# joesharratt1229/DT4Image_Restoration

Hardware: AMD Instinct MI355X
Metric: pnp_admm_iterations_per_sec (higher is better)
Workload: dtype f32

## Files before the change

dt4image_restoration_amd/_lib.py:

```python
from __future__ import annotations

import ctypes as C
import os

_HERE = os.path.dirname(os.path.abspath(__file__))
LIB_PATH = os.environ.get("PNP_LIB_PATH") or os.path.join(_HERE, "csrc", "libpnpadmm.so")

PNP_FLAG_PROFILE = 1
PNP_FLAG_NO_DENOISER = 2
PNP_FLAG_KEEP_STAGES = 4
PNP_FLAG_BF16_CONVS = 8
PNP_FLAG_PROFILE_LAYERS = 16
PNP_SSIM_CLAMP_X = 1
PNP_RES_COLS = 6
PNP_RES_DELTA = 1
PNP_RES_DC = 2
RESIDUAL_COLUMNS = ("primal", "dx", "dz", "du", "delta", "dc")
PNP_MC_MAX_COILS = 32
PNP_MC_MAX_CG = 64
PNP_CC_MAX_COILS = 64
PNP_PW_MAX_COILS = 64
PNP_ESPIRIT_MAX_COILS = 16
PNP_ESPIRIT_MAX_KSIZE = 8
PNP_ESPIRIT_MAX_N = 512
PNP_TV_MAX_ITERS = 64
PNP_PRIOR_UNET = 0
PNP_PRIOR_TV = 1
PRIORS = {"unet": PNP_PRIOR_UNET, "tv": PNP_PRIOR_TV}
PNP_SENS_BOX = 0
PNP_SENS_HANN = 1
SENS_WINDOWS = {"box": PNP_SENS_BOX, "hann": PNP_SENS_HANN}
PROFILE_CLASSES = 6
PROFILE_CLASS_NAMES = ("conv3x3_mfma", "conv_first", "conv_last", "fft_rows", "fft_cols_prox", "other")
N_LAYERS = 28


class pnp_config(C.Structure):
    _fields_ = [("n", C.c_int32), ("h", C.c_int32), ("w", C.c_int32), ("device", C.c_int32), ("flags", C.c_int32)]


_vp, _fp, _u8p = C.c_void_p, C.c_void_p, C.c_void_p

SIGNATURES = {
    "pnp_create": (C.c_int, [C.POINTER(pnp_config), C.POINTER(C.c_void_p)]),
    "pnp_destroy": (C.c_int, [C.c_void_p]),
    "pnp_last_error": (C.c_char_p, []),
    "pnp_version": (C.c_char_p, []),
    "pnp_load_unet_weights": (C.c_int, [C.c_void_p, C.c_void_p, C.c_size_t]),
    "pnp_reset": (C.c_int, [C.c_void_p, _fp, _fp, _u8p, C.c_int, _fp, _fp, _fp, _vp]),
    "pnp_set_kspace": (C.c_int, [C.c_void_p, _fp, _u8p, C.c_int, _vp]),
    "pnp_step": (C.c_int, [C.c_void_p, _fp, _fp, _fp, _fp, _fp, _fp, _fp, _u8p, _vp]),
    "pnp_denoise": (C.c_int, [C.c_void_p, _fp, _fp, _fp, _vp]),
    "pnp_tv_denoise": (C.c_int, [C.c_void_p, _fp, _fp, C.c_int, _fp, _vp]),
    "pnp_set_prior": (C.c_int, [C.c_void_p, C.c_int, C.c_double, C.c_int]),
    "pnp_get_prior": (C.c_int, [C.c_void_p, C.POINTER(C.c_int), C.POINTER(C.c_double), C.POINTER(C.c_int)]),
    "pnp_fft2c": (C.c_int, [C.c_void_p, _fp, _fp, C.c_int, C.c_int, C.c_int, C.c_int, _vp]),
    "pnp_prox_dual": (C.c_int, [C.c_void_p, _fp, _fp, _fp, _fp, _fp, _vp]),
    "pnp_psnr": (C.c_int, [C.c_void_p, _fp, _fp, _fp, _vp]),
    "pnp_ssim": (C.c_int, [C.c_void_p, _fp, _fp, C.c_float, C.c_float, C.c_float, C.c_int, C.c_int, _fp, _fp, _vp]),
    "pnp_residuals": (C.c_int, [C.c_void_p, _fp, _fp, _fp, _vp, C.c_int, _fp, _vp]),
    "pnp_acquire": (C.c_int, [C.c_void_p, _fp, _u8p, C.c_int, C.c_double, C.c_uint64, C.c_int, _fp, _fp, _fp, _vp]),
    "pnp_set_kspace_mc": (C.c_int, [C.c_void_p, _fp, _fp, C.c_int, C.c_int, _u8p, C.c_int, C.c_int, _vp]),
    "pnp_reset_mc": (C.c_int, [C.c_void_p, _fp, _fp, _fp, C.c_int, C.c_int, _u8p, C.c_int, C.c_int, _fp, _fp, _fp, _vp]),
    "pnp_mc_coils": (C.c_int, [C.c_void_p]),
    "pnp_mc_cg_residual": (C.c_int, [C.c_void_p, _fp, _vp]),
    "pnp_mc_normal": (C.c_int, [C.c_void_p, _fp, _fp, _fp, _vp]),
    "pnp_acquire_mc": (C.c_int, [C.c_void_p, _fp, _fp, C.c_int, C.c_int, _u8p, C.c_int, C.c_double, C.c_uint64, C.c_int, _fp, _fp, _fp, _vp]),
    "pnp_estimate_sens": (C.c_int, [C.c_void_p, _fp, C.c_int, C.c_int, C.c_int, C.c_int, C.c_double, C.c_int, _fp, _fp, _vp]),
    "pnp_coil_compress_matrix": (C.c_int, [C.c_void_p, _fp, C.c_int, C.c_int, C.c_int, C.c_int, _fp, _fp, _fp, _vp]),
    "pnp_coil_compress_apply": (C.c_int, [C.c_void_p, _fp, C.c_int, _fp, C.c_int, C.c_int, _fp, _vp]),
    "pnp_noise_cov": (C.c_int, [C.c_void_p, _fp, C.c_int, C.c_int, C.c_int, C.c_int, _fp, _vp]),
    "pnp_whiten_matrix": (C.c_int, [C.c_void_p, _fp, C.c_int, C.c_int, C.c_int, _fp, _fp, _fp, _vp]),
    "pnp_whiten_apply": (C.c_int, [C.c_void_p, _fp, C.c_int, _fp, C.c_int, _fp, _vp]),
    "pnp_espirit_sens": (C.c_int, [C.c_void_p, _fp, C.c_int, C.c_int, C.c_int, C.c_int, C.c_double, C.c_double, C.c_int, C.c_int, C.c_double,
                                  C.c_int, _fp, _fp, _fp, _vp, _vp]),
    "pnp_snapshot_bytes": (C.c_size_t, [C.c_void_p]),
    "pnp_snapshot": (C.c_int, [C.c_void_p, _fp, _fp, _fp, _fp, _vp, _vp]),
    "pnp_restore": (C.c_int, [C.c_void_p, _vp, _fp, _fp, _fp, _fp, _vp]),
    "pnp_unet_read_stage": (C.c_int, [C.c_void_p, C.c_int, _fp, C.POINTER(C.c_int), C.POINTER(C.c_int),
                                      C.POINTER(C.c_int), _vp]),
    "pnp_profile_reset": (C.c_int, [C.c_void_p]),
    "pnp_profile_collect": (C.c_int, [C.c_void_p, C.POINTER(C.c_double), C.POINTER(C.c_int64)]),
    "pnp_profile_layers": (C.c_int, [C.c_void_p, C.POINTER(C.c_double), C.POINTER(C.c_int64)]),
    "pnp_conv_algorithms": (C.c_int, [C.c_void_p, C.POINTER(C.c_int32)]),
    "pnp_bf16_weight_terms": (C.c_int, [C.c_void_p]),
    "pnp_workspace_bytes": (C.c_size_t, [C.c_void_p]),
}

_lib = None


class PnPError(RuntimeError):
    pass


def load() -> C.CDLL:
    global _lib
    if _lib is not None:
        return _lib
    if not os.path.exists(LIB_PATH):
        raise PnPError(f"{LIB_PATH} not found: build it with `python -c 'import __graft_entry__ as g; g.build()'` "
                       f"or `make -C {os.path.dirname(LIB_PATH)}`; there is no CPU fallback")
    lib = C.CDLL(LIB_PATH)
    for name, (res, args) in SIGNATURES.items():
        fn = getattr(lib, name)
        fn.restype = res
        fn.argtypes = args
    _lib = lib
    return lib


def check(rc: int, what: str) -> None:
    if rc != 0:
        msg = load().pnp_last_error()
        raise PnPError(f"{what} failed ({rc}): {msg.decode() if msg else '?'}")
```

dt4image_restoration_amd/csrc/conv_kernels.hip:

```cpp
#include "pnp_internal.h"
#include "conv_staging.h"
#include <cstring>
#include <cstdlib>

namespace pnp {



const LayerSpec kLayers[N_LAYERS] = {
    {2, 32, 3, 0, SRC_SIGMA, 0},    {32, 32, 3, 0, SRC_PLAIN, 0},   {32, 32, 3, 0, SRC_PLAIN, 0},
    {32, 64, 3, 1, SRC_POOL, 0},    {64, 64, 3, 1, SRC_PLAIN, 0},   {64, 64, 3, 1, SRC_PLAIN, 0},
    {64, 128, 3, 2, SRC_POOL, 0},   {128, 128, 3, 2, SRC_PLAIN, 0}, {128, 128, 3, 2, SRC_PLAIN, 0},
    {128, 256, 3, 3, SRC_POOL, 0},  {256, 256, 3, 3, SRC_PLAIN, 0}, {256, 256, 3, 3, SRC_PLAIN, 0},
    {256, 512, 3, 4, SRC_POOL, 0},  {512, 512, 3, 4, SRC_PLAIN, 0}, {512, 512, 3, 4, SRC_PLAIN, 0},
    {768, 256, 3, 3, SRC_UPCAT, 256}, {256, 256, 3, 3, SRC_PLAIN, 0}, {256, 256, 3, 3, SRC_PLAIN, 0},
    {384, 128, 3, 2, SRC_UPCAT, 128}, {128, 128, 3, 2, SRC_PLAIN, 0}, {128, 128, 3, 2, SRC_PLAIN, 0},
    {192, 64, 3, 1, SRC_UPCAT, 64},  {64, 64, 3, 1, SRC_PLAIN, 0},   {64, 64, 3, 1, SRC_PLAIN, 0},
    {96, 32, 3, 0, SRC_UPCAT, 32},   {32, 32, 3, 0, SRC_PLAIN, 0},   {32, 32, 3, 0, SRC_PLAIN, 0},
    {32, 1, 1, 0, SRC_PLAIN, 0},
};

ConvPlan conv3x3_plan(int N, int H, int W, int Cin, int Cout, bool bf16, int src_mode, bool allow_ws) {
    ConvPlan p{};
    p.tw = W >= 32 ? 32 : (W >= 16 ? 16 : 8);
// ... 553 lines not shown
                for (unsigned z0 = 0; z0 < nz; z0 += 4) {
                    float4 q[4][4];
#pragma unroll
                    for (int k = 0; k < 4; ++k) {
                        const unsigned z = z0 + k < nz ? z0 + k : nz - 1;
#pragma unroll
                        for (int j = 0; j < 4; ++j)
                            q[k][j] = __builtin_bit_cast(float4, __builtin_amdgcn_raw_buffer_load_b128(prsrc, e[j] * 4u, (int)(z * pstride), 16));
                    }
#pragma unroll
                    for (int k = 0; k < 4; ++k)
                        if (z0 + k < nz) {
#pragma unroll
                            for (int j = 0; j < 4; ++j) { sum[j].x += q[k][j].x; sum[j].y += q[k][j].y; sum[j].z += q[k][j].z; sum[j].w += q[k][j].w; }
                        }
                }
#pragma unroll
                for (int j = 0; j < 4; ++j) {
                    if (!ok[j]) continue;
                    float4 v = sum[j];
                    v.x = fmaxf(v.x, kLeaky * v.x); v.y = fmaxf(v.y, kLeaky * v.y);
                    v.z = fmaxf(v.z, kLeaky * v.z); v.w = fmaxf(v.w, kLeaky * v.w);
                    *reinterpret_cast<float4*>(a.dst + e[j]) = v;
                }
            }
        }
    }
}

__global__ __launch_bounds__(256) void splitk_reduce_kernel(const float* __restrict__ partial, const float* __restrict__ bias,
                                                            float* __restrict__ dst, const float* __restrict__ tact,
                                                            size_t plane4, int splitk, int cout4, size_t slice4) {
    for (size_t i = (size_t)blockIdx.x * 256 + threadIdx.x; i < plane4; i += (size_t)gridDim.x * 256) {
        if (tact != nullptr && tact[i / slice4] > 0.5f) continue;
        float4 s = reinterpret_cast<const float4*>(bias)[i % cout4];
        for (int z0 = 0; z0 < splitk; z0 += 8) {
            float4 p[8];
#pragma unroll
            for (int k = 0; k < 8; ++k) p[k] = reinterpret_cast<const float4*>(partial)[(size_t)(z0 + k < splitk ? z0 + k : splitk - 1) * plane4 + i];
#pragma unroll
            for (int k = 0; k < 8; ++k)
                if (z0 + k < splitk) { s.x += p[k].x; s.y += p[k].y; s.z += p[k].z; s.w += p[k].w; }
        }
        s.x = fmaxf(s.x, kLeaky * s.x); s.y = fmaxf(s.y, kLeaky * s.y);
        s.z = fmaxf(s.z, kLeaky * s.z); s.w = fmaxf(s.w, kLeaky * s.w);
        reinterpret_cast<float4*>(dst)[i] = s;
    }
}

template <int TW, int MT, int NT, int WM, int WN, int CK, int SRC, bool SPLITK, int BF16>
static hipError_t launch_inst(const ConvArgs& a, const ConvPlan& p, hipStream_t s) {
    constexpr int WPS = (MT * NT <= 2 && SRC != SRC_UPCAT) ? 3 : (MT * NT <= 8 ? 2 : 1);
    constexpr int WPS16 = (MT * NT <= 2 && BF16 == 2) ? 3 : WPS;
    dim3 grid((unsigned)(p.tiles_x * p.tiles_y * a.N), (unsigned)(a.Cout / p.bn), (unsigned)p.splitk);
    constexpr bool CAN16 = BF16 != 0 && !SPLITK && MT == 2 && NT == 1 && WM == 4 && CK == 32 && SRC != SRC_POOL;
    if constexpr (CAN16) {
        if (a.act16 & 1) {
            hipLaunchKernelGGL((conv3x3_mfma_kernel<TW, MT, NT, WM, WN, CK, SRC, WPS16, SPLITK, BF16, true>), grid, dim3(256), 0, s, a);
            return hipGetLastError();
        }
    }
    if (a.act16 != 0) return hipErrorInvalidValue;
    hipLaunchKernelGGL((conv3x3_mfma_kernel<TW, MT, NT, WM, WN, CK, SRC, WPS, SPLITK, BF16, false>), grid, dim3(256), 0, s, a);
    return hipGetLastError();
}

template <int TW, int MT, int NT, int WM, int WN, int CK, bool SPLITK, int BF16>
static hipError_t launch_cfg(const ConvArgs& a, const ConvPlan& p, int src_mode, hipStream_t s) {
    switch (src_mode) {
        case SRC_PLAIN: return launch_inst<TW, MT, NT, WM, WN, CK, SRC_PLAIN, SPLITK, BF16>(a, p, s);
        case SRC_POOL:  return launch_inst<TW, MT, NT, WM, WN, CK, SRC_POOL, SPLITK, BF16>(a, p, s);
        case SRC_UPCAT: return launch_inst<TW, MT, NT, WM, WN, CK, SRC_UPCAT, SPLITK, BF16>(a, p, s);
        default: return hipErrorInvalidValue;
    }
}

template <int TW, int BF16>
static hipError_t launch_tw(const ConvArgs& a, const ConvPlan& p, int src_mode, hipStream_t s) {
    if constexpr (BF16 == 0) {
        if (p.mt == 1 && p.wn == 4) return launch_cfg<TW, 1, 1, 1, 4, 16, true, 0>(a, p, src_mode, s);
        if (p.mt == 1 && p.wn == 2) return launch_cfg<TW, 1, 1, 2, 2, 16, true, 0>(a, p, src_mode, s);
    }
    if (p.mt == 2 && p.wn == 4) return launch_cfg<TW, 2, 1, 1, 4, 32, true, BF16>(a, p, src_mode, s);
    if (p.mt == 2 && p.wn == 2) return launch_cfg<TW, 2, 1, 2, 2, 32, true, BF16>(a, p, src_mode, s);
    if constexpr (BF16 == 0) {
        if (p.nt == 1 && p.mt == 1) return launch_cfg<TW, 1, 1, 4, 1, 32, false, 0>(a, p, src_mode, s);
    }
    if (p.nt == 1) return launch_cfg<TW, 2, 1, 4, 1, 32, false, BF16>(a, p, src_mode, s);
    if (p.nt == 2 && p.wn == 1) return launch_cfg<TW, 4, 2, 4, 1, 16, false, BF16>(a, p, src_mode, s);
    if (p.nt == 2) return launch_cfg<TW, 4, 2, 2, 2, 32, false, BF16>(a, p, src_mode, s);
    if constexpr (BF16 != 0) return hipErrorInvalidValue;
    else return launch_cfg<TW, 4, 4, 2, 2, 32, false, 0>(a, p, src_mode, s);
}

hipError_t launch_conv3x3(const ConvArgs& a0, const ConvPlan& p, int src_mode, hipStream_t s) {
    if (a0.Cin % 32 != 0 || a0.Cout % 32 != 0 || (a0.Cout > 64 && a0.Cout % 128 != 0)) return hipErrorInvalidValue;
    if (!conv3x3_tensor_fits(a0.N, a0.H, a0.W, a0.Cin, a0.Cout)) return hipErrorInvalidValue;
    if (p.ws) return launch_conv3x3_bf16ws(a0, p, src_mode, s);
    ConvArgs a = a0;
    a.tilesX = p.tiles_x;
    a.tilesY = p.tiles_y;
    const bool split = p.mt <= 2 && p.wn >= 2;
    if (split && a.partial == nullptr) return hipErrorInvalidValue;
    if (!split || (size_t)p.tiles_x * p.tiles_y * a.N * (a.Cout / p.bn) > 4096) a.arrive = nullptr;
    hipError_t e;
    if (a.bf16 == 2) {
        if (p.tw == 32) e = launch_tw<32, 2>(a, p, src_mode, s);
        else if (p.tw == 16) e = launch_tw<16, 2>(a, p, src_mode, s);
        else e = launch_tw<8, 2>(a, p, src_mode, s);
    } else if (a.bf16 == 1) {
        if (p.tw == 32) e = launch_tw<32, 1>(a, p, src_mode, s);
        else if (p.tw == 16) e = launch_tw<16, 1>(a, p, src_mode, s);
        else e = launch_tw<8, 1>(a, p, src_mode, s);
    } else {
        if (p.tw == 32) e = launch_tw<32, 0>(a, p, src_mode, s);
        else if (p.tw == 16) e = launch_tw<16, 0>(a, p, src_mode, s);
        else e = launch_tw<8, 0>(a, p, src_mode, s);
    }
    if (e != hipSuccess || !split || a.arrive != nullptr) return e;
    const size_t plane4 = (size_t)a.N * a.H * a.W * a.Cout / 4;
    unsigned blocks = (unsigned)((plane4 + 255) / 256);
    if (blocks > 2048u) blocks = 2048u;
    hipLaunchKernelGGL(splitk_reduce_kernel, dim3(blocks), dim3(256), 0, s, a.partial, a.bias, a.dst, a.tact, plane4,
                       p.splitk, a.Cout / 4, (size_t)a.H * a.W * a.Cout / 4);
    return hipGetLastError();
}

bool conv3x3_tensor_fits(int N, int H, int W, int Cin, int Cout) {
    (void)Cin;
    return (size_t)N * H * W * (size_t)Cout * 4 < ((size_t)1 << 31);
}

bool conv3x3_pooled_output_ok(const ConvPlan& p) {
    return p.splitk == 1 && p.mt <= 2 && p.nt == 1 && p.wm == 4;
}

size_t conv3x3_partial_floats(const ConvPlan& p, int N, int H, int W, int Cout) {
    return (p.mt <= 2 && p.wn >= 2) ? (size_t)p.splitk * N * H * W * Cout : 0;
}

Tuning tuning_from_env() {
    Tuning t;
    if (const char* v = getenv("PNP_WINO_MIN_CIN")) t.wino_min_cin = atoi(v);
    if (const char* v = getenv("PNP_WINO_MIN_BLOCKS")) t.wino_min_blocks = atol(v);
    t.wino_big = getenv("PNP_WINO_BIG_GROUPS") != nullptr;
    t.wino_small = getenv("PNP_WINO_SMALL_GROUPS") != nullptr;
    t.no_wino = getenv("PNP_NO_WINOGRAD") != nullptr;
    if (const char* v = getenv("PNP_WINO_F4_MIN_CIN")) t.f4_min_cin = atoi(v);
    t.no_f4 = getenv("PNP_NO_WINO_F4") != nullptr;
    t.no_f4_phased = getenv("PNP_NO_WINO_F4_PHASED") != nullptr;
    t.no_f4_fused_last = getenv("PNP_NO_F4_FUSED_LAST") != nullptr;
    t.no_f4_fused_first = getenv("PNP_NO_F4_FUSED_FIRST") != nullptr;
    if (const char* v = getenv("PNP_WINO_F4_MT16")) t.f4_mt16 = atoi(v);
    if (const char* v = getenv("PNP_WINO_F4_ORDER")) t.f4_order = atoi(v) != 0;
    t.bf16_f32_acts = getenv("PNP_BF16_F32_ACTS") != nullptr;
    t.bf16_no_ws = getenv("PNP_BF16_NO_WS") != nullptr;
    t.bf16_w1 = getenv("PNP_BF16_W1") != nullptr;
    t.bf16_no_holdhi = getenv("PNP_BF16_NO_HOLDHI") != nullptr;
    t.fft_xcd = getenv("PNP_FFT_XCD") != nullptr && atoi(getenv("PNP_FFT_XCD")) != 0;
    if (const char* v = getenv("PNP_SPLITK_INLAUNCH")) t.splitk_inlaunch = atoi(v);
    if (const char* v = getenv("PNP_SLICE128_MIN_N")) t.slice128_min_n = atoi(v);
    return t;
}

hipError_t raise_lds_cap(const void* fn, int bytes, DeviceOnce& once) {
    int dev = 0;
    hipError_t e = hipGetDevice(&dev);
    if (e != hipSuccess) return e;
    const uint64_t bit = 1ull << (dev & 63);
    if (once.mask.load(std::memory_order_relaxed) & bit) return hipSuccess;
    e = hipFuncSetAttribute(fn, hipFuncAttributeMaxDynamicSharedMemorySize, bytes);
    if (e != hipSuccess) return e;
    once.mask.fetch_or(bit, std::memory_order_relaxed);
    return hipSuccess;
}

__global__ __launch_bounds__(256) void conv_first_kernel(const float* __restrict__ ximg, const float2* __restrict__ z,
                                                         const float2* __restrict__ u, const float* __restrict__ sigma,
                                                         const float* __restrict__ tact, const float* __restrict__ w,
                                                         const float* __restrict__ bias, float* __restrict__ dst,
                                                         int N, int H, int W, int tilesX, int tilesY, int TYG, int dst16) {
    constexpr int TH = 8, TW = 32, PW = TW + 2, PH = TH + 2;
    __shared__ float dt[2][PH][PW + 1];
    __shared__ float mt[2][PH][PW + 1];
    const int groupsY = (tilesY + TYG - 1) / TYG;
    int bt = blockIdx.x;
    const int tx0 = (bt % tilesX) * TW;
    bt /= tilesX;
    const int tyg = bt % groupsY;
    const int n = bt / groupsY;
    if (tact != nullptr && tact[n] > 0.5f) return;
    auto stage = [&](int buf, int ty0) {
        for (int i = threadIdx.x; i < PH * PW; i += 256) {
            const int py = i / PW, px = i % PW;
            const int gy = ty0 + py - 1, gx = tx0 + px - 1;
            float d = 0.f, m = 0.f;
            if (gy >= 0 && gy < H && gx >= 0 && gx < W) {
                const size_t q = ((size_t)n * H + gy) * W + gx;
                d = ximg != nullptr ? ximg[q] : (z[q].x - u[q].x);
                m = 1.f;
            }
            dt[buf][py][px] = d;
            mt[buf][py][px] = m;
        }
    };
    const int t_first = tyg * TYG, t_last = min(t_first + TYG, tilesY);
    stage(0, t_first * TH);
    const int cg = threadIdx.x & 7, col = threadIdx.x >> 3;
    float wd[4][9], ws[4][9], br[4], brs[4];
    const float sg = sigma[n];
#pragma unroll
    for (int j = 0; j < 4; ++j) {
        br[j] = bias[cg * 4 + j];
        brs[j] = br[j];
#pragma unroll
        for (int k = 0; k < 9; ++k) {
            wd[j][k] = w[(cg * 4 + j) * 18 + k];
            ws[j][k] = w[(cg * 4 + j) * 18 + 9 + k] * sg;
            brs[j] += ws[j][k];
        }
    }
    const int gx = tx0 + col;
    for (int t = t_first; t < t_last; ++t) {
        const int buf = (t - t_first) & 1, ty0 = t * TH;
        const bool interior = tx0 > 0 && tx0 + TW < W && ty0 > 0 && ty0 + TH < H;
        __syncthreads();
        if (t + 1 < t_last) stage(buf ^ 1, ty0 + TH);
        float d[3][3], m[3][3];
#pragma unroll
        for (int r = 0; r < 2; ++r)
#pragma unroll
            for (int c = 0; c < 3; ++c) { d[r + 1][c] = dt[buf][r][col + c]; m[r + 1][c] = mt[buf][r][col + c]; }
#pragma unroll
        for (int row = 0; row < TH; ++row) {
#pragma unroll
            for (int c = 0; c < 3; ++c) {
                d[0][c] = d[1][c]; d[1][c] = d[2][c]; d[2][c] = dt[buf][row + 2][col + c];
                m[0][c] = m[1][c]; m[1][c] = m[2][c]; m[2][c] = mt[buf][row + 2][col + c];
            }
            float acc[4];
            if (interior) {
#pragma unroll
                for (int j = 0; j < 4; ++j) acc[j] = brs[j];
#pragma unroll
                for (int ky = 0; ky < 3; ++ky)
#pragma unroll
                    for (int kx = 0; kx < 3; ++kx)
#pragma unroll
                        for (int j = 0; j < 4; ++j) acc[j] = fmaf(wd[j][ky * 3 + kx], d[ky][kx], acc[j]);
            } else {
#pragma unroll
                for (int j = 0; j < 4; ++j) acc[j] = br[j];
#pragma unroll
                for (int ky = 0; ky < 3; ++ky)
#pragma unroll
                    for (int kx = 0; kx < 3; ++kx)
#pragma unroll
                        for (int j = 0; j < 4; ++j) {
                            acc[j] = fmaf(wd[j][ky * 3 + kx], d[ky][kx], acc[j]);
                            acc[j] = fmaf(ws[j][ky * 3 + kx], m[ky][kx], acc[j]);
                        }
            }
            const int gy = ty0 + row;
            if (gy < H && gx < W) {
                float4 o;
                o.x = fmaxf(acc[0], kLeaky * acc[0]);
                o.y = fmaxf(acc[1], kLeaky * acc[1]);
                o.z = fmaxf(acc[2], kLeaky * acc[2]);
                o.w = fmaxf(acc[3], kLeaky * acc[3]);
                if (dst16) {
                    uint2 o16;
                    o16.x = __builtin_bit_cast(unsigned, __builtin_convertvector((f32x2){o.x, o.y}, bf16x2));
                    o16.y = __builtin_bit_cast(unsigned, __builtin_convertvector((f32x2){o.z, o.w}, bf16x2));
                    *reinterpret_cast<uint2*>(reinterpret_cast<uint16_t*>(dst) + (((size_t)n * H + gy) * W + gx) * 32 + cg * 4) = o16;
                } else {
                    *reinterpret_cast<float4*>(dst + (((size_t)n * H + gy) * W + gx) * 32 + cg * 4) = o;
                }
            }
        }
    }
}

hipError_t launch_conv_first(const float* ximg, const float2* z, const float2* u, const float* sigma,
                             const float* tact, const float* w, const float* bias, float* dst, int N, int H, int W,
                             hipStream_t s, bool dst_bf16) {
    const int tilesX = (W + 31) / 32, tilesY = (H + 7) / 8;
    int tyg = 8;
    while (tyg > 1 && (long)tilesX * ((tilesY + tyg - 1) / tyg) * N < 512) tyg >>= 1;
    const int groupsY = (tilesY + tyg - 1) / tyg;
    hipLaunchKernelGGL(conv_first_kernel, dim3((unsigned)(tilesX * groupsY * N)), dim3(256), 0, s, ximg, z, u, sigma, tact, w,
                       bias, dst, N, H, W, tilesX, tilesY, tyg, dst_bf16 ? 1 : 0);
    return hipGetLastError();
}

__global__ __launch_bounds__(256) void conv_last_kernel(const float* __restrict__ act, const float* __restrict__ ximg,
                                                        const float2* __restrict__ z, const float2* __restrict__ u,
                                                        const float* __restrict__ tact, const float* __restrict__ w,
                                                        const float* __restrict__ bias, float* __restrict__ out,
                                                        int N, int H, int W) {
    const int cg = threadIdx.x & 7;
    const float4 wv = *reinterpret_cast<const float4*>(w + cg * 4);
    const float b = bias[0];
    const size_t hw = (size_t)H * W;
    const size_t total = (size_t)N * hw;
    for (size_t p = (size_t)blockIdx.x * 32 + (threadIdx.x >> 3); p < total; p += (size_t)gridDim.x * 32) {
        const int n = (int)(p / hw);
// ... 45 lines not shown
```

dt4image_restoration_amd/csrc/denoiser_plan.hip:

```cpp
#include "denoiser_plan.h"

#include <cstdio>

namespace pnp {

namespace {

constexpr int kStageLayers = 3;
constexpr int kFirstLayer = 0, kLastLayer = N_LAYERS - 1;
constexpr int kHead = kFirstLayer + 1;
constexpr int kTail = kLastLayer - 1;

bool is_wino(const ConvLaunch& l) { return l.family == FAM_WINO2 || l.family == FAM_WINO4; }

bool pooled_copy_ok(const pnp_config& cfg, const ConvLaunch& l) {
    const int lh = cfg.h >> kLayers[l.layer].level, lw = cfg.w >> kLayers[l.layer].level;
    return lh % 2 == 0 && lw % 2 == 0 && (is_wino(l) || conv3x3_pooled_output_ok(l.conv));
}

}

bool plan_denoiser(const pnp_config& cfg, const Tuning& tune, DenoiserPlan* out, std::string* err) {
    DenoiserPlan& P = *out;
    P = DenoiserPlan{};
    const bool bf16 = (cfg.flags & PNP_FLAG_BF16_CONVS) != 0;
    const bool keep_stages = (cfg.flags & PNP_FLAG_KEEP_STAGES) != 0;
    P.bf16_terms = bf16 ? (tune.bf16_w1 ? 1 : 2) : 0;
    if (cfg.flags & PNP_FLAG_NO_DENOISER) return true;

    ConvLaunch rec[N_LAYERS] = {};
    int first_up = N_LAYERS;
    for (int li = N_LAYERS - 1; li >= 0; --li) if (kLayers[li].src == SRC_UPCAT) first_up = li;
    for (int li = 0; li < N_LAYERS; ++li) {
        const LayerSpec& L = kLayers[li];
        ConvLaunch& r = rec[li];
        r.layer = li;
        r.src_mode = L.src;
        const int pos = li % kStageLayers;
        if (li != kLastLayer) r.dst = {L.level, pos == 0 ? SLOT_PING : (pos == 1 ? SLOT_PONG : (li < first_up ? SLOT_SKIP : SLOT_PING))};
        if (li == kFirstLayer) continue;
        if (L.src == SRC_UPCAT) { r.src0 = {L.level, SLOT_SKIP}; r.src1 = rec[li - 1].dst; }
        else r.src0 = rec[li - 1].dst;
    }
    rec[kFirstLayer].family = FAM_FIRST;
    rec[kLastLayer].family = FAM_LAST;

    for (int li = kHead; li <= kTail; ++li) {
        const LayerSpec& L = kLayers[li];
        ConvLaunch& r = rec[li];
        const int lh = cfg.h >> L.level, lw = cfg.w >> L.level;
        if (L.src == SRC_POOL && pooled_copy_ok(cfg, rec[li - 1])) {
            r.src_mode = SRC_PLAIN;
            rec[li - 1].pooled = r.src0 = {kLayers[li - 1].level, SLOT_POOL};
            P.pool_ok[kLayers[li - 1].level] = true;
        }
        r.wino = winograd_plan(cfg.n, lh, lw, L.cin, L.cout, r.src_mode, tune);
        if (li == kTail && r.wino.algo == 4 && !keep_stages && (tune.no_f4_fused_last || r.wino.bn != 32 || r.wino.mt != 32)) {
            Tuning t2 = tune;
            t2.no_f4 = true;
            r.wino = winograd_plan(cfg.n, lh, lw, L.cin, L.cout, r.src_mode, t2);
        }
        const bool ws_ok = !tune.bf16_no_ws && (r.src_mode != SRC_UPCAT || upsample_lines_regular(lh));
        r.conv = conv3x3_plan(cfg.n, lh, lw, L.cin, L.cout, bf16, r.src_mode, ws_ok);
        r.conv.holdhi = tune.bf16_no_holdhi ? 0 : 1;
        if (li == kTail && r.conv.nt == 1 && (P.bf16_terms != 2 || tune.bf16_no_holdhi)) r.conv.ws = 0;
        r.family = (r.wino.use && !bf16) ? (r.wino.algo == 4 ? FAM_WINO4 : FAM_WINO2) : (r.conv.ws ? FAM_WS : FAM_DIRECT);
        if (r.family == FAM_WINO4) continue;
        if (!conv3x3_tensor_fits(cfg.n, lh, lw, L.cin, L.cout)) {
            char buf[512];
            snprintf(buf, sizeof buf, "pnp_create: layer %d's output tensor (%d x %d x %d x %d floats) reaches 2 GiB, past this "
                     "kernel's buffer descriptor: use a smaller batch per handle", li, cfg.n, lh, lw, L.cout);
            *err = buf;
            return false;
        }
        if (is_wino(r)) continue;
        const size_t f = conv3x3_partial_floats(r.conv, cfg.n, lh, lw, L.cout);
        if (f > P.partial_floats) P.partial_floats = f;
    }
    P.want_arrive = P.partial_floats > 0 && tune.splitk_inlaunch;

    P.fuse_last = !keep_stages && (is_wino(rec[kTail]) || conv3x3_pooled_output_ok(rec[kTail].conv));
    P.fuse_first = rec[kHead].family == FAM_WINO4 && rec[kHead].wino.bn == 32 && rec[kHead].wino.mt == 32 && !tune.no_f4_fused_first;
    if (P.fuse_first) { rec[kHead].fused_first = true; rec[kHead].src_mode = SRC_FIRST; }
    rec[kTail].fused_last = P.fuse_last;

    int src0_from[N_LAYERS] = {}, skip_reader[N_LAYERS] = {};
    for (int li = kHead; li <= kLastLayer; ++li) {
        int w = li - 1;
        while (w > 0 && !(rec[w].dst == rec[li].src0) && !(rec[w].pooled == rec[li].src0)) --w;
        src0_from[li] = w;
        if (kLayers[li].src == SRC_UPCAT) skip_reader[w] = li;
    }

    P.act16 = bf16 && !keep_stages && !tune.bf16_f32_acts && P.pool_ok[0];
    for (int li = kHead; li <= kTail; ++li)
        if (kLayers[li].level == 0) P.act16 = P.act16 && conv3x3_pooled_output_ok(rec[li].conv);
    if (P.act16) {
        auto can = [&](int li) { return li >= kHead && li <= kTail && (kLayers[li].level == 0 || rec[li].conv.ws != 0); };
        bool out16[N_LAYERS] = {};
        out16[kFirstLayer] = true;
        for (int li = kHead; li < kTail; ++li) {
            if (kLayers[li + 1].src == SRC_UPCAT) continue;
            const bool next_reads = rec[li + 1].src0 == rec[li].dst;
            out16[li] = can(li) && (!next_reads || can(li + 1)) && (skip_reader[li] == 0 || can(skip_reader[li]));
        }
        for (int li = kHead; li <= kTail; ++li) {
            const bool in16 = rec[li].src0.slot == SLOT_POOL ? false : out16[src0_from[li]];
            if (kLayers[li].level == 0 && !in16) out16[li] = false;
            rec[li].act16 = (in16 ? 1 : 0) | (out16[li] ? 2 : 0);
        }
        rec[kFirstLayer].act16 = 2;
        for (int li = kHead; li < kTail; ++li) {
            ConvLaunch &w = rec[li], &r = rec[li + 1];
            if (kLayers[li].level == 0 && w.pooled.slot == SLOT_POOL && (w.act16 & 2) && w.conv.ws && r.conv.ws && w.conv.holdhi && P.bf16_terms == 2) {
                w.act16 |= 4;
                r.act16 |= 1;
            }
        }
    }

    for (int li = kFirstLayer; li <= kTail; ++li) {
        const LayerSpec& L = kLayers[li];
        const size_t bytes = (size_t)cfg.n * (cfg.h >> L.level) * (cfg.w >> L.level) * L.cout * sizeof(float);
        P.plane_bytes[L.level][rec[li].dst.slot] = bytes;
        if (kLayers[li + 1].src == SRC_POOL) P.plane_bytes[L.level][SLOT_POOL] = bytes / 4;
    }
    for (int s = 0; s < N_STAGES; ++s) {
        const ConvLaunch& r = rec[kStageLayers * s + kStageLayers - 1];
        const LayerSpec& L = kLayers[r.layer];
        P.stage[s] = {r.dst, L.cout, cfg.h >> L.level, cfg.w >> L.level, (r.act16 & 2) != 0, r.fused_last};
    }
    for (int li = 0; li < N_LAYERS; ++li) {
        P.family[li] = rec[li].family;
        const bool fused = (li == kFirstLayer && P.fuse_first) || (li == kLastLayer && P.fuse_last);
        P.launch_of[li] = fused ? -1 : P.n_launches;
        if (!fused) P.launch[P.n_launches++] = rec[li];
    }
    return true;
}

}
```

dt4image_restoration_amd/csrc/pnp_capi.hip:

```cpp
#include "../../include/pnpadmm.h"
#include "pnp_internal.h"
#include "denoiser_plan.h"
#include "block_reduce.h"

#include <cmath>
#include <cstdarg>
#include <cstdio>
#include <cstring>
#include <cstdlib>
#include <initializer_list>
#include <new>
#include <string>
#include <vector>

using namespace pnp;

namespace {

thread_local std::string g_err;

int fail(int code, const char* fmt, ...) {
    char buf[512];
    va_list ap;
    va_start(ap, fmt);
// ... 1171 lines not shown

int pnp_whiten_apply(pnp_handle e, const float* in, int coils, const float* wmat, int wmat_n, float* out, void* stream) {
    PNP_API_BEGIN
    const char* fn = "pnp_whiten_apply";
    if (coils < 1 || coils > PNP_PW_MAX_COILS) return fail(PNP_ERR_INVALID, "%s: coils must be 1..%d (got %d)", fn, PNP_PW_MAX_COILS, coils);
    if (wmat_n < 1) return fail(PNP_ERR_INVALID, "%s: wmat_n must be 1 or the handle's n (got %d)", fn, wmat_n);
    if (!in) return fail(PNP_ERR_INVALID, "%s: null in", fn);
    if (!wmat) return fail(PNP_ERR_INVALID, "%s: null wmat", fn);
    if (!out) return fail(PNP_ERR_INVALID, "%s: null out", fn);
    if (out == wmat || in == wmat) return fail(PNP_ERR_INVALID, "%s: wmat must not alias in or out", fn);
    const uintptr_t pi = (uintptr_t)in, po = (uintptr_t)out;
    const uintptr_t gap = pi < po ? po - pi : pi - po;
    if (gap != 0 && gap < (uintptr_t)2048 * (uintptr_t)coils)
        return fail(PNP_ERR_INVALID, "%s: out must be in exactly (in place) or must not overlap it (the buffers lie %zu bytes apart)", fn, (size_t)gap);
    if (!e) return fail(PNP_ERR_INVALID, "%s: null handle", fn);
    const int N = e->cfg.n, H = e->cfg.h, W = e->cfg.w;
    if (wmat_n != 1 && wmat_n != N) return fail(PNP_ERR_INVALID, "%s: wmat_n must be 1 or the handle's n=%d (got %d)", fn, N, wmat_n);
    if (N > 65535) return fail(PNP_ERR_INVALID, "%s: n must be <= 65535 (got %d)", fn, N);
    const uintptr_t bytes = (uintptr_t)N * coils * H * W * sizeof(float2), wbytes = (uintptr_t)wmat_n * coils * coils * sizeof(float2);
    if (gap != 0 && gap < bytes)
        return fail(PNP_ERR_INVALID, "%s: out must be in exactly (in place) or must not overlap it (the buffers lie %zu bytes apart)", fn, (size_t)gap);
    const uintptr_t pw = (uintptr_t)wmat;
    if ((pw < po + bytes && po < pw + wbytes) || (pw < pi + bytes && pi < pw + wbytes))
        return fail(PNP_ERR_INVALID, "%s: wmat must not alias in or out", fn);
    PNP_ON_DEVICE(e);
    hipStream_t s = (hipStream_t)stream;
    Prof p(e, s, PROF_OTHER, -1);
    HIP_TRY(launch_prewhiten_apply((const float2*)in, (const float2*)wmat, wmat_n, coils, (float2*)out, N, H, W, s));
    return PNP_OK;
    PNP_API_END("pnp_whiten_apply")
}

int pnp_espirit_sens(pnp_handle e, const float* y0, int coils, int acs_h, int acs_w, int ksize, double sv_thresh, double crop, int iters,
                     int window, double thresh, int flags, float* sens, float* eval, float* kern, int32_t* nkept, void* stream) {
    PNP_API_BEGIN
    const char* fn = "pnp_espirit_sens";
    if (flags != 0) return fail(PNP_ERR_INVALID, "%s: flags must be 0 (got 0x%x)", fn, (unsigned)flags);
    if (!(thresh >= 0.0) || !(thresh < 1.0)) return fail(PNP_ERR_INVALID, "%s: thresh must be finite and in [0, 1) (got %g)", fn, thresh);
    if (!(crop >= 0.0) || !(crop < 1.0)) return fail(PNP_ERR_INVALID, "%s: crop must be finite and in [0, 1) (got %g)", fn, crop);
    if (!(sv_thresh > 0.0) || !(sv_thresh < 1.0)) return fail(PNP_ERR_INVALID, "%s: sv_thresh must be in (0, 1) (got %g)", fn, sv_thresh);
    if (iters < 1 || iters > 64) return fail(PNP_ERR_INVALID, "%s: iters must be 1..64 (got %d)", fn, iters);
    if (window != PNP_SENS_BOX && window != PNP_SENS_HANN)
        return fail(PNP_ERR_INVALID, "%s: window must be PNP_SENS_BOX or PNP_SENS_HANN (got %d)", fn, window);
    if (coils < 1 || coils > PNP_ESPIRIT_MAX_COILS)
        return fail(PNP_ERR_INVALID, "%s: coils must be 1..%d (got %d); compress more channels first", fn, PNP_ESPIRIT_MAX_COILS, coils);
    if (ksize < 2 || ksize > PNP_ESPIRIT_MAX_KSIZE) return fail(PNP_ERR_INVALID, "%s: ksize must be 2..%d (got %d)", fn, PNP_ESPIRIT_MAX_KSIZE, ksize);
    if (coils * ksize * ksize > PNP_ESPIRIT_MAX_N)
        return fail(PNP_ERR_INVALID, "%s: coils * ksize^2 must be <= %d (got %d * %d^2)", fn, PNP_ESPIRIT_MAX_N, coils, ksize);
    if (acs_h < ksize || (acs_h & 1)) return fail(PNP_ERR_INVALID, "%s: acs_h must be even and >= ksize=%d (got %d)", fn, ksize, acs_h);
    if (acs_w < ksize || (acs_w & 1)) return fail(PNP_ERR_INVALID, "%s: acs_w must be even and >= ksize=%d (got %d)", fn, ksize, acs_w);
    if (!y0) return fail(PNP_ERR_INVALID, "%s: null y0", fn);
    if (!sens) return fail(PNP_ERR_INVALID, "%s: null sens", fn);
    if (sens == y0) return fail(PNP_ERR_INVALID, "%s: sens must not alias y0", fn);
    if (!e) return fail(PNP_ERR_INVALID, "%s: null handle", fn);
    const int N = e->cfg.n, H = e->cfg.h, W = e->cfg.w;
    if (acs_h > H) return fail(PNP_ERR_INVALID, "%s: acs_h must be <= h=%d (got %d)", fn, H, acs_h);
    if (acs_w > W) return fail(PNP_ERR_INVALID, "%s: acs_w must be <= w=%d (got %d)", fn, W, acs_w);
    if (int rc = check_kspace_sizes(fn, e)) return rc;
    if ((long long)N * coils > 65535) return fail(PNP_ERR_INVALID, "%s: n * coils must be <= 65535 (got %d * %d)", fn, N, coils);
    PNP_ON_DEVICE(e);
    hipStream_t s = (hipStream_t)stream;
    int rc;
    const size_t np = (size_t)espirit_padded(coils, ksize), D = (size_t)(2 * ksize - 1);
    const size_t mat_bytes = (size_t)N * 2 * np * np * sizeof(double2), kern_bytes = (size_t)N * coils * coils * D * D * sizeof(float2);
    if ((rc = cm_ensure(e, true))) return rc;
    if ((rc = es_ensure(e, mat_bytes + kern_bytes + (size_t)N * 8))) return rc;
    double2* const ws = (double2*)e->es_ws;
    float2* const R = kern ? (float2*)kern : (float2*)((char*)e->es_ws + mat_bytes);
    int* const nk = nkept ? (int*)nkept : (int*)((char*)e->es_ws + mat_bytes + kern_bytes);
    float* const smax = e->cm_max + (size_t)N * pixel_chunks(H, W);
    {
        Prof p(e, s, PROF_OTHER, -1);
        HIP_TRY(launch_espirit_gram((const float2*)y0, coils, acs_h, acs_w, ksize, ws, N, H, W, s));
        HIP_TRY(launch_espirit_eig(ws, coils, ksize, N, s));
        HIP_TRY(launch_espirit_kern(ws, coils, ksize, sv_thresh, R, nk, N, s));
        p.end(3);
    }
    {
        Prof p(e, s, PROF_OTHER, -1);
        HIP_TRY(launch_coilmap_window((const float2*)y0, (float2*)sens, acs_h, acs_w, window == PNP_SENS_HANN, N, coils, H, W, s));
    }
    if ((rc = plain_fft2(e, (float2*)sens, (float2*)sens, N * coils, 1, s))) return rc;
    Prof p(e, s, PROF_OTHER, -1);
    HIP_TRY(launch_coilmap_rss((const float2*)sens, coils, e->cm_rss, e->cm_max, N, H, W, s));
    HIP_TRY(launch_coilmap_max(e->cm_max, smax, N, H, W, s));
    HIP_TRY(launch_espirit_pixels((float2*)sens, R, e->cm_rss, smax, coils, ksize, iters, (float)crop, (float)thresh, eval, N, H, W, s));
    p.end(3);
    return PNP_OK;
    PNP_API_END("pnp_espirit_sens")
}

size_t pnp_snapshot_bytes(pnp_handle e) {
    return e ? SnapLayout(e).bytes() : 0;
}

int pnp_snapshot(pnp_handle e, const float* x, const float* z, const float* u, const float* t_state, void* dst,
                 void* stream) {
    PNP_API_BEGIN
    if (!e || !x || !z || !u || !dst) return fail(PNP_ERR_INVALID, "pnp_snapshot: null argument");
    PNP_ON_DEVICE(e);
    const SnapLayout snap(e);
    char* d = static_cast<char*>(dst);
    hipStream_t s = (hipStream_t)stream;
    HIP_TRY(hipMemcpyAsync(d, x, snap.x_bytes(), hipMemcpyDeviceToDevice, s));
    HIP_TRY(hipMemcpyAsync(d + snap.z_off(), z, snap.zu_bytes(), hipMemcpyDeviceToDevice, s));
    HIP_TRY(hipMemcpyAsync(d + snap.u_off(), u, snap.zu_bytes(), hipMemcpyDeviceToDevice, s));
    if (t_state) HIP_TRY(hipMemcpyAsync(d + snap.t_off(), t_state, snap.t_bytes(), hipMemcpyDeviceToDevice, s));
    else HIP_TRY(hipMemsetAsync(d + snap.t_off(), 0, snap.t_bytes(), s));
    return PNP_OK;
    PNP_API_END("pnp_snapshot")
}

int pnp_restore(pnp_handle e, const void* src, float* x, float* z, float* u, float* t_state, void* stream) {
    PNP_API_BEGIN
    if (!e || !x || !z || !u || !src) return fail(PNP_ERR_INVALID, "pnp_restore: null argument");
    PNP_ON_DEVICE(e);
    const SnapLayout snap(e);
    const char* d = static_cast<const char*>(src);
    hipStream_t s = (hipStream_t)stream;
    HIP_TRY(hipMemcpyAsync(x, d, snap.x_bytes(), hipMemcpyDeviceToDevice, s));
    HIP_TRY(hipMemcpyAsync(z, d + snap.z_off(), snap.zu_bytes(), hipMemcpyDeviceToDevice, s));
    HIP_TRY(hipMemcpyAsync(u, d + snap.u_off(), snap.zu_bytes(), hipMemcpyDeviceToDevice, s));
    if (t_state) HIP_TRY(hipMemcpyAsync(t_state, d + snap.t_off(), snap.t_bytes(), hipMemcpyDeviceToDevice, s));
    return PNP_OK;
    PNP_API_END("pnp_restore")
}

int pnp_unet_read_stage(pnp_handle e, int which, float* dst, int* c, int* hh, int* ww, void* stream) {
    PNP_API_BEGIN
    if (!e || which < 0 || which > 8) return fail(PNP_ERR_INVALID, "pnp_unet_read_stage: which must be 0..8");
    if (e->cfg.flags & PNP_FLAG_NO_DENOISER) return fail(PNP_ERR_STATE, "pnp_unet_read_stage: handle has no denoiser");
    const StagePlan& st = e->dplan.stage[which];
    if (st.fused_away) return fail(PNP_ERR_STATE, "pnp_unet_read_stage: stage 8 is fused away; create the handle with PNP_FLAG_KEEP_STAGES");
    if (st.bf16) return fail(PNP_ERR_STATE, "pnp_unet_read_stage: this stage is held as bf16 on this handle; create it with PNP_FLAG_KEEP_STAGES");
    PNP_ON_DEVICE(e);
    const float* src = e->plane[st.plane.level][st.plane.slot];
    if (c) *c = st.c;
    if (hh) *hh = st.h;
    if (ww) *ww = st.w;
    if (dst) HIP_TRY(launch_nhwc_to_nchw(src, dst, e->cfg.n, st.c, st.h, st.w, (hipStream_t)stream));
    return PNP_OK;
    PNP_API_END("pnp_unet_read_stage")
}

int pnp_conv_algorithms(pnp_handle e, int32_t* algo28) {
    PNP_API_BEGIN
    if (!e || !algo28) return fail(PNP_ERR_INVALID, "pnp_conv_algorithms: null argument");
    if (e->cfg.flags & PNP_FLAG_NO_DENOISER) return fail(PNP_ERR_STATE, "pnp_conv_algorithms: handle has no denoiser");
    for (int i = 0; i < N_LAYERS; ++i) algo28[i] = e->dplan.family[i];
    return PNP_OK;
    PNP_API_END("pnp_conv_algorithms")
}

int pnp_profile_reset(pnp_handle e) {
    PNP_API_BEGIN
    if (!e) return fail(PNP_ERR_INVALID, "null handle");
    e->ev_used = 0;
    memset(e->cls_ms, 0, sizeof e->cls_ms); memset(e->cls_n, 0, sizeof e->cls_n);
    memset(e->layer_ms, 0, sizeof e->layer_ms); memset(e->layer_n, 0, sizeof e->layer_n);
    return PNP_OK;
    PNP_API_END("pnp_profile_reset")
}

int pnp_profile_collect(pnp_handle e, double* total_ms, int64_t* launches) {
    PNP_API_BEGIN
    if (!e) return fail(PNP_ERR_INVALID, "null handle");
    PNP_ON_DEVICE(e);
    for (size_t i = 0; i < e->ev_used; ++i) {
        float ms = 0.f;
        HIP_TRY(hipEventElapsedTime(&ms, e->events[i].a, e->events[i].b));
        const EventPair& p = e->events[i];
        e->cls_ms[p.cls] += ms; e->cls_n[p.cls] += p.count;
        if (p.layer >= 0) { e->layer_ms[p.layer] += ms; e->layer_n[p.layer] += 1; }
    }
    e->ev_used = 0;
    for (int i = 0; i < PNP_PROFILE_CLASSES; ++i) {
        if (total_ms) total_ms[i] = e->cls_ms[i];
        if (launches) launches[i] = e->cls_n[i];
    }
    return PNP_OK;
    PNP_API_END("pnp_profile_collect")
}

int pnp_profile_layers(pnp_handle e, double* layer_ms, int64_t* layer_launches) {
    PNP_API_BEGIN
    if (!e) return fail(PNP_ERR_INVALID, "null handle");
    for (int i = 0; i < N_LAYERS; ++i) {
        if (layer_ms) layer_ms[i] = e->layer_ms[i];
        if (layer_launches) layer_launches[i] = e->layer_n[i];
    }
    return PNP_OK;
    PNP_API_END("pnp_profile_layers")
}

}
```

dt4image_restoration_amd/csrc/pnp_internal.h:

```cpp
#pragma once
#include <hip/hip_runtime.h>
#include <stdint.h>
#include <stddef.h>
#include <atomic>
#include <vector>

namespace pnp {

struct Tuning {
    int wino_min_cin = 32;
    long wino_min_blocks = 192;
    bool wino_big = false;
    bool wino_small = false;
    bool no_wino = false;
    int f4_min_cin = 32;
    bool no_f4 = false;
    bool no_f4_fused_first = false;
    bool no_f4_fused_last = false;
    bool no_f4_phased = false;
    int f4_mt16 = 0;
    bool bf16_no_ws = false;
    bool bf16_f32_acts = false;
    bool bf16_no_holdhi = false;
    bool bf16_w1 = false;
    int f4_order = 1;
    int splitk_inlaunch = 0;
    bool fft_xcd = false;
    int slice128_min_n = 192;
};
Tuning tuning_from_env();

struct DeviceOnce { std::atomic<uint64_t> mask{0}; };
hipError_t raise_lds_cap(const void* fn, int bytes, DeviceOnce& once);

enum SrcMode : int { SRC_PLAIN = 0, SRC_SIGMA = 1, SRC_POOL = 2, SRC_UPCAT = 3, SRC_FIRST = 4 };

struct LayerSpec {
    int cin, cout, ksize, level, src, cskip;
};
static constexpr int N_LAYERS = 28;
extern const LayerSpec kLayers[N_LAYERS];

struct ConvArgs {
    const float* src0;
    const float* src1;
    const float* wpack;
    const float* bias;
    float* dst;
    float* pooled;
    const float* last_w; const float* last_b; const float* last_ximg; const float2* last_z; const float2* last_u; float* last_out;
    const float* first_w; const float* first_b; const float* first_sigma;
    float* partial;
    unsigned* arrive;
    const float* tact;
    int N, H, W;
    int Cin, Cskip, Cout;
    int tilesX, tilesY;
    float rh, rw;
    int bf16;
    int act16;
    int order;
#ifdef PNP_STAMPS
    int stamp_slot;
#endif
#ifdef PNP_DIAG
    int diag;
#endif
};

struct ConvPlan {
    int tw, th;
    int bm, bn;
    int mt, nt, wm, wn;
    int ck;
    int splitk;
    int ws;
    int holdhi = 1;
    int tiles_x, tiles_y;
};
ConvPlan conv3x3_plan(int N, int H, int W, int Cin, int Cout, bool bf16 = false, int src_mode = SRC_PLAIN, bool allow_ws = true);
hipError_t launch_conv3x3_bf16ws(const ConvArgs& a, const ConvPlan& p, int src_mode, hipStream_t s);
size_t conv3x3_partial_floats(const ConvPlan& p, int N, int H, int W, int Cout);
bool conv3x3_pooled_output_ok(const ConvPlan& p);
bool conv3x3_tensor_fits(int N, int H, int W, int Cin, int Cout);
hipError_t launch_conv3x3(const ConvArgs& a, const ConvPlan& p, int src_mode, hipStream_t s);

size_t conv3x3_pack_floats(int cin, int cout);
void pack_conv3x3_weights(const float* oihw, int cin, int cout, int ck, float* dst);
size_t conv3x3_pack_floats_bf16(int cin, int cout, int terms);
void pack_conv3x3_weights_bf16(const float* oihw, int cin, int cout, int ck, int terms, float* dst);

struct WinoPlan {
    bool use;
    int algo;
    int tw, th, bn, wm, wn, ck, tiles_x, tiles_y;
    int stack;
    int mt;
    int phased;
    int order;
};
WinoPlan winograd_plan(int N, int H, int W, int Cin, int Cout, int src_mode, const Tuning& t);
bool upsample_lines_regular(int H);
size_t winograd4_pack_floats(int cin, int cout);
void pack_winograd4_weights(const float* oihw, int cin, int cout, int ck, float* dst);
hipError_t launch_conv3x3_winograd4(const ConvArgs& a, const WinoPlan& p, int src_mode, hipStream_t s);
size_t winograd_pack_floats(int cin, int cout);
void pack_winograd_weights(const float* oihw, int cin, int cout, int ck, float* dst);
hipError_t launch_conv3x3_winograd(const ConvArgs& a, const WinoPlan& p, int src_mode, hipStream_t s);

hipError_t launch_conv_first(const float* ximg, const float2* z, const float2* u, const float* sigma,
                             const float* tact, const float* w, const float* bias, float* dst,
                             int N, int H, int W, hipStream_t s, bool dst_bf16 = false);
hipError_t launch_conv_last(const float* act, const float* ximg, const float2* z, const float2* u,
                            const float* tact, const float* w, const float* bias, float* out,
                            int N, int H, int W, hipStream_t s);
hipError_t launch_nhwc_to_nchw(const float* src, float* dst, int N, int C, int H, int W, hipStream_t s);

struct FftPlan {
    int h, w;
    float2* tw_h;
    float2* tw_w;
};

bool kspace_len_ok(int L);
hipError_t launch_fft_rows(const float2* in, float2* out, const float2* tw, int batch, int H, int W, int inverse, int shift, hipStream_t s);
hipError_t launch_fft_cols(float2* data, const float2* tw, int batch, int H, int W, int inverse, int shift, hipStream_t s);
hipError_t launch_fft_rows_real(const float* x, float2* work, const float2* tw, int N, int H, int W, hipStream_t s);
hipError_t launch_fft_rows_fwd_admm(const float* x, const float2* u, float2* work, const float2* tw, const float* tact, int N, int H, int W,
                                    hipStream_t s);
hipError_t launch_fft_cols_prox(float2* work, const float2* tw, const float2* y0s, const uint8_t* masks, int mask_n, const float* mu,
                                const float* tact, int N, int H, int W, hipStream_t s);
hipError_t launch_fft_rows_inv_admm(const float2* work, const float* x, float2* z, float2* u, const float2* tw, const float* tact, int N,
                                    int H, int W, hipStream_t s);
namespace mixed {
hipError_t launch_fft_rows(const float2* in, float2* out, const float2* tw, int batch, int H, int W, int inverse, int shift, hipStream_t s);
hipError_t launch_fft_cols(float2* data, const float2* tw, int batch, int H, int W, int inverse, int shift, hipStream_t s);
hipError_t launch_fft_rows_real(const float* x, float2* work, const float2* tw, int N, int H, int W, hipStream_t s);
hipError_t launch_fft_rows_fwd_admm(const float* x, const float2* u, float2* work, const float2* tw, const float* tact, int N, int H, int W,
                                    hipStream_t s);
hipError_t launch_fft_cols_prox(float2* work, const float2* tw, const float2* y0s, const uint8_t* masks, int mask_n, const float* mu,
                                const float* tact, int N, int H, int W, hipStream_t s);
hipError_t launch_fft_rows_inv_admm(const float2* work, const float* x, float2* z, float2* u, const float2* tw, const float* tact, int N,
                                    int H, int W, hipStream_t s);
}

hipError_t launch_admm_slice128(const float* x, float2* z, float2* u, const float2* tw, const float2* y0s,
                                const uint8_t* masks, int mask_n, const float* mu, const float* tact, int N, hipStream_t s);

hipError_t launch_reset(const float2* x0, const float2* y0, const uint8_t* mask, int mask_n, float* x, float2* z,
                        float2* u, float2* y0s, uint8_t* masks, int N, int H, int W, hipStream_t s);
hipError_t launch_finish(const float* tact, float* tstate, uint8_t* done, int N, hipStream_t s);
size_t admm_xcd_counter_bytes();
bool admm_xcd_usable(int N, int H, int W);
hipError_t launch_admm_xcd(const float* x, float2* z, float2* u, float2* work, const float2* tw, const float2* y0s,
                           const uint8_t* masks, int mask_n, const float* mu, const float* tact, unsigned* ctr, unsigned epoch, int N, int H, hipStream_t s);
hipError_t launch_psnr(const float* x, const float* gt, float* out, int N, int HW, hipStream_t s);

static constexpr int kSsimMaxRadius = 16;
struct SsimArgs {
    const float* x;
    const float* gt;
    float* map;
    double* partial;
    float* out;
    int H, W;
    int radius;
    int clamp_x;
    float c1, c2;
    float w[2 * kSsimMaxRadius + 1];
};
int ssim_tiles(int H, int W);
hipError_t launch_ssim(const SsimArgs& a, int N, hipStream_t s);

hipError_t launch_residual_tiles(const float* x, const float2* z, const float2* u, const float* xp, const float2* zp, const float2* up,
                                 double* partial, int N, int H, int W, hipStream_t s);
hipError_t launch_misfit_tiles(const float2* fx, const float2* y0s, const uint8_t* masks, int mask_n, double* dcpartial, int N, int H, int W,
                               hipStream_t s);
hipError_t launch_residual_reduce(const double* partial, const double* dcpartial, int has_delta, int has_dc, float* out, int N, int H, int W,
                                  hipStream_t s);

hipError_t launch_acquire_epilogue(float2* work, const uint8_t* mask, int mask_n, float2* y0, double sigma, uint64_t seed, int N, int H, int W,
                                   hipStream_t s, int coils = 1);
hipError_t launch_acquire_clamp(const float2* aty0, float2* x0, int N, int H, int W, hipStream_t s);

hipError_t launch_sense_expand(const float2* src, const float* src_real, const float2* sens, int sens_n, int C, const float* tact, float2* work,
                               int N, int H, int W, hipStream_t s);
hipError_t launch_sense_mask(float2* work, const uint8_t* masks, int mask_n, int C, int N, int H, int W, hipStream_t s);
hipError_t launch_sense_combine(const float2* work, const float2* sens, int sens_n, int C, const float2* pv, const float* mu, const float* tact,
                                float2* q, double* partial, int N, int H, int W, hipStream_t s);
hipError_t launch_sense_cg_init(const float2* aty, const float* x, const float2* u, const float2* q, const float* mu, const float* tact, float2* r,
                                float2* pv, double* partial, int N, int H, int W, hipStream_t s);
hipError_t launch_sense_scalar(const double* partial, int mode, const float* tact, double* sc, int N, int H, int W, hipStream_t s);
hipError_t launch_sense_cg_update(float2* z, float2* r, const float2* pv, const float2* q, const double* sc, const float* tact, double* partial,
                                  int N, int H, int W, hipStream_t s);
hipError_t launch_sense_cg_dir(const float2* r, float2* pv, const double* sc, const float* tact, int N, int H, int W, hipStream_t s);
hipError_t launch_sense_dual(const float* x, const float2* z, float2* u, const float* tact, int N, int H, int W, hipStream_t s);
hipError_t launch_sense_cgres(const double* sc, float* out, int N, hipStream_t s);
hipError_t launch_sense_misfit(const float2* fx, const float2* ys, const uint8_t* masks, int mask_n, int C, double* dcpartial, int N, int H, int W,
                               hipStream_t s);
hipError_t launch_sense_install(const float2* y, const uint8_t* mask, int mask_n, int C, float2* ys, float2* work, uint8_t* masks, int N, int H,
                                int W, hipStream_t s);
hipError_t launch_sense_iterate(const float2* x0, float* x, float2* z, float2* u, int N, int H, int W, hipStream_t s);

hipError_t launch_coilmap_window(const float2* y, float2* sens, int acs_h, int acs_w, int hann, int N, int C, int H, int W, hipStream_t s);
hipError_t launch_coilmap_rss(const float2* l, int C, float* rss, float* partial, int N, int H, int W, hipStream_t s);
hipError_t launch_coilmap_max(const float* partial, float* smax, int N, int H, int W, hipStream_t s);
hipError_t launch_coilmap_normalise(float2* l, int C, const float* rss, const float* smax, float thresh, int N, int H, int W, hipStream_t s);

static constexpr int kGramMinBins = 1024, kGramMaxChunks = 64;
inline int gram_chunk_len(long long count) {
    const long long per = ((count + kGramMaxChunks - 1) / kGramMaxChunks + 31) / 32 * 32;
    return per < kGramMinBins ? kGramMinBins : (int)per;
}
inline int gram_chunks(long long count) { return (int)((count + gram_chunk_len(count) - 1) / gram_chunk_len(count)); }
hipError_t launch_coilcomp_gram(const float2* y, int C, int acs_h, int acs_w, double2* partial, double2* gram, int N, int H, int W, hipStream_t s);
hipError_t launch_coilcomp_eig(const double2* gram, int C, float2* cmat, float* eig, int N, hipStream_t s);
hipError_t launch_coilcomp_apply(const float2* in, const float2* cmat, int cmat_n, int C, int V, float2* out, int N, int H, int W, hipStream_t s);

hipError_t launch_prewhiten_cov(const float2* noise, int noise_n, int C, int S, double2* partial, double2* psi, hipStream_t s);
hipError_t launch_prewhiten_chol(const double2* psi, int psi_n, int C, float2* wmat, float2* lmat, int* info, hipStream_t s);
hipError_t launch_prewhiten_apply(const float2* in, const float2* wmat, int wmat_n, int C, float2* out, int N, int H, int W, hipStream_t s);

inline int espirit_padded(int C, int k) { return (C * k * k + 1) & ~1; }
hipError_t launch_espirit_gram(const float2* y, int C, int acs_h, int acs_w, int k, double2* ws, int N, int H, int W, hipStream_t s);
hipError_t launch_espirit_eig(double2* ws, int C, int k, int N, hipStream_t s);
hipError_t launch_espirit_kern(const double2* ws, int C, int k, double sv_thresh, float2* kern, int* nkept, int N, hipStream_t s);
hipError_t launch_espirit_pixels(float2* sens, const float2* kern, const float* rss, const float* smax, int C, int k, int iters, float crop,
                                 float thresh, float* eval, int N, int H, int W, hipStream_t s);

static constexpr int kTvT = 10, kTvRegion = 128, kTvTile = kTvRegion - 2 * kTvT - 1;
struct TvArgs {
    const float* v;
    const float2* z;
    const float2* u;
    const float* lam;
    float scale;
    const float* tact;
    const float2* p_in;
    float2* p_out;
    float* out;
    int H, W;
    int iters;
    int tiles_x, tiles_y;
};
hipError_t launch_tv_fused(TvArgs a, int N, hipStream_t s);
hipError_t launch_tv_iter(TvArgs a, int N, hipStream_t s);
hipError_t launch_tv_close(TvArgs a, int N, hipStream_t s);

}
```

dt4image_restoration_amd/csrc/winograd4_kernels.hip:

```cpp
#include "pnp_internal.h"
#include "conv_staging.h"
#include <type_traits>

namespace pnp {

#ifdef PNP_STAMPS
#define W4_SLOTS 32
#define W4_WGS 1024
#define W4_N 16
__device__ unsigned long long g_w4_stamps[W4_SLOTS * W4_WGS * W4_N];
static int g_w4_slot = 0;
#define W4T() __builtin_amdgcn_s_memtime()
#endif

namespace {
constexpr double kA = 0.75, kB = 1.5;
constexpr float fA = 0.75f, fB = 1.5f, fA2 = 0.5625f, fB2 = 2.25f, fA3 = 0.421875f, fB3 = 3.375f;
constexpr float fK0 = 1.265625f;
constexpr float fK1 = 2.8125f;

__device__ __forceinline__ float4 f4add(float4 a, float4 b) { return make_float4(a.x + b.x, a.y + b.y, a.z + b.z, a.w + b.w); }
typedef float v2f __attribute__((ext_vector_type(2)));
typedef float f32x4 __attribute__((ext_vector_type(4)));

template <int G>
__device__ __forceinline__ void bt3(const v2f* d, v2f* o) {
    if constexpr (G == 0) {
        o[0] = fK0 * d[0] + (d[4] - fK1 * d[2]);
        const v2f e = d[4] - fB2 * d[2];
        const v2f od = fA * (d[3] - fB2 * d[1]);
        o[1] = e + od;
        o[2] = e - od;
    } else {
        const v2f e = d[4] - fA2 * d[2];
        const v2f od = fB * (d[3] - fA2 * d[1]);
        o[0] = e + od;
        o[1] = e - od;
        o[2] = fK0 * d[1] + (d[5] - fK1 * d[3]);
    }
}

template <int QJ, int PW, int CKP, int PLANE>
__device__ __forceinline__ void wino4_input_transform(const float* w, float* v) {
    constexpr int X0 = QJ == 0 ? 0 : 1;
    v2f c[6][3];
#pragma unroll
    for (int y = 0; y < 6; ++y) {
        v2f d[6];
        __builtin_amdgcn_sched_barrier(0);
#pragma unroll
        for (int x = 0; x < 5; ++x) d[X0 + x] = *reinterpret_cast<const v2f*>(w + (y * PW + X0 + x) * CKP);
        bt3<QJ>(d, c[y]);
    }
#pragma unroll
    for (int j = 0; j < 3; ++j) {
        const v2f r0 = c[0][j], r1 = c[1][j], r2 = c[2][j], r3 = c[3][j], r4 = c[4][j], r5 = c[5][j];
        float* vj = v + (3 * QJ + j) * PLANE;
        *reinterpret_cast<v2f*>(vj + 0 * 6 * PLANE) = fK0 * r0 + (r4 - fK1 * r2);
        const v2f e1 = r4 - fB2 * r2, o1 = fA * (r3 - fB2 * r1);
        *reinterpret_cast<v2f*>(vj + 1 * 6 * PLANE) = e1 + o1;
        *reinterpret_cast<v2f*>(vj + 2 * 6 * PLANE) = e1 - o1;
        const v2f e2 = r4 - fA2 * r2, o2 = fB * (r3 - fA2 * r1);
        *reinterpret_cast<v2f*>(vj + 3 * 6 * PLANE) = e2 + o2;
        *reinterpret_cast<v2f*>(vj + 4 * 6 * PLANE) = e2 - o2;
        *reinterpret_cast<v2f*>(vj + 5 * 6 * PLANE) = fK0 * r1 + (r5 - fK1 * r3);
    }
}
}

constexpr int kW4Tail = 8 * 64 * 4;
size_t winograd4_pack_floats(int cin, int cout) { return (size_t)cout * cin * 36 + (size_t)(cout / 16) * kW4Tail; }

void pack_winograd4_weights(const float* oihw, int cin, int cout, int ck, float* dst) {
    const int CK = ck, S = CK / 4;
    const double pts[5] = {0.0, kA, -kA, kB, -kB};
    double G[6][3];
    for (int j = 0; j < 5; ++j) {
        double nrm = 1.0;
        for (int l = 0; l < 5; ++l) if (l != j) nrm *= pts[j] - pts[l];
        G[j][0] = 1.0 / nrm; G[j][1] = pts[j] / nrm; G[j][2] = pts[j] * pts[j] / nrm;
    }
    G[5][0] = 0.0; G[5][1] = 0.0; G[5][2] = 1.0;
    std::vector<float> U((size_t)cout * cin * 36);
    for (int co = 0; co < cout; ++co)
        for (int ci = 0; ci < cin; ++ci) {
            const float* g = oihw + ((size_t)co * cin + ci) * 9;
            double t[6][3];
            for (int i = 0; i < 6; ++i)
                for (int kx = 0; kx < 3; ++kx) t[i][kx] = G[i][0] * g[kx] + G[i][1] * g[3 + kx] + G[i][2] * g[6 + kx];
            for (int i = 0; i < 6; ++i)
                for (int j = 0; j < 6; ++j)
                    U[((size_t)co * cin + ci) * 36 + 6 * i + j] = (float)(t[i][0] * G[j][0] + t[i][1] * G[j][1] + t[i][2] * G[j][2]);
        }
    size_t o = 0;
    for (int cb = 0; cb < cout / 16; ++cb) {
        for (int ch = 0; ch < cin / CK; ++ch)
            for (int xi = 0; xi < 36; ++xi)
                for (int l = 0; l < 64; ++l)
                    for (int sidx = 0; sidx < S; ++sidx) {
                        const int co = 16 * cb + (l & 15);
                        const int ci = CK * ch + S * (l >> 4) + sidx;
                        dst[o++] = U[((size_t)co * cin + ci) * 36 + xi];
                    }
        for (int i = 0; i < kW4Tail; ++i) dst[o++] = 0.f;
    }
}

bool upsample_lines_regular(int H) {
    if (H < 2 || H % 2) return false;
    const int Hs = H / 2;
    const float rh = (float)(Hs - 1) / (float)(H - 1);
    for (int g = 0; g < H; ++g) {
        const float sc = rh * (float)g;
        const int i0 = (int)sc;
        const int i1 = i0 + (i0 < Hs - 1 ? 1 : 0);
        const float l = sc - (float)i0;
        const int s0 = g >= 1 ? (g - 1) / 2 : -1;
        if (l < 1.f && i0 != s0 && i0 != s0 + 1) return false;
        if (l > 0.f && i1 != s0 && i1 != s0 + 1) return false;
    }
    return true;
}

__device__ __forceinline__ void wino4_decode(int bid, int ny, int ntiles, int order, int& cby, int& bt) {
    if (order == 0) {
        const int grp = bid / (8 * ny), rem = bid % (8 * ny);
        cby = rem >> 3;
        bt = grp * 8 + (rem & 7);
    } else {
        const int xcd = bid & 7, slot = bid >> 3;
        const int tpx = (ntiles + 7) >> 3;
        const int lt = slot / ny;
        cby = slot - lt * ny;
        bt = lt < tpx ? xcd * tpx + lt : ntiles;
    }
}

template <int CTRL>
__device__ __forceinline__ float dpp_xchg(float v) {
    return __builtin_bit_cast(float, __builtin_amdgcn_update_dpp(0, __builtin_bit_cast(int, v), CTRL, 0xF, 0xF, false));
}
template <int H, int CTRL>
__device__ __forceinline__ void row_reduce_scatter_step(v2f* P, bool bit) {
#pragma unroll
    for (int i = 0; i < H; ++i) {
        const v2f lo = P[i], hi = P[i + H];
        const v2f keep = bit ? hi : lo, send = bit ? lo : hi;
        P[i] = v2f{keep.x + dpp_xchg<CTRL>(send.x), keep.y + dpp_xchg<CTRL>(send.y)};
    }
}

template <int TW, bool STK, int MT = 32, bool FUSE = false>
__device__ __forceinline__ void wino4_epilogue(const ConvArgs& a, const f32x4 (&acc)[36], int n, int th, int tg, int cl, int cb,
                                               int tx0, int ty0, bool live, float* xch = nullptr) {
    constexpr int TC = TW / 4, TR = MT / TC;
    constexpr unsigned OOB = 0x80000000u;
    const int cout0 = cb * 16 + cl;
    const float bias = a.bias[cout0];
    const int Hp = a.H >> 1, Wp = a.W >> 1;
    auto at6 = [&](v2f m0, v2f m1, v2f m2, v2f m3, v2f m4, v2f m5, v2f* t) {
        const v2f s1 = m1 + m2, d1 = m1 - m2, s2 = m3 + m4, d2 = m3 - m4;
        t[0] = m0 + s1 + s2;
        t[1] = fA * d1 + fB * d2;
        t[2] = fA2 * s1 + fB2 * s2;
        t[3] = fA3 * d1 + fB3 * d2 + m5;
    };
    if (!live) return;
    const bool fused = FUSE && a.last_w != nullptr;
#ifdef PNP_DIAG
    const bool nostore = (a.diag & 1) != 0;
#else
    constexpr bool nostore = false;
#endif
    v2f part[2];
    const __amdgpu_buffer_rsrc_t rdst = __builtin_amdgcn_make_buffer_rsrc(
        (void*)(a.dst + (size_t)(n + (STK ? th : 0)) * a.H * a.W * a.Cout), 0, nostore ? 0 : a.H * a.W * a.Cout * 4, 0x00020000);
    const __amdgpu_buffer_rsrc_t rpool = __builtin_amdgcn_make_buffer_rsrc(
        (void*)(a.pooled != nullptr ? a.pooled + (size_t)(n + (STK ? th : 0)) * Hp * Wp * a.Cout : a.dst), 0,
        (a.pooled != nullptr && !nostore) ? Hp * Wp * a.Cout * 4 : 0, 0x00020000);
#pragma unroll
    for (int rp = 0; rp < 2; ++rp) {
        v2f T[4][6];
#pragma unroll
        for (int j = 0; j < 6; ++j) {
            v2f m[6];
#pragma unroll
            for (int i = 0; i < 6; ++i) m[i] = v2f{acc[6 * i + j][2 * rp], acc[6 * i + j][2 * rp + 1]};
            v2f t[4];
            at6(m[0], m[1], m[2], m[3], m[4], m[5], t);
#pragma unroll
            for (int ay = 0; ay < 4; ++ay) T[ay][j] = t[ay];
        }
        v2f Y[4][4];
#pragma unroll
        for (int ay = 0; ay < 4; ++ay) {
            at6(T[ay][0], T[ay][1], T[ay][2], T[ay][3], T[ay][4], T[ay][5], Y[ay]);
#pragma unroll
            for (int ax = 0; ax < 4; ++ax) {
                const v2f sv = Y[ay][ax] + bias;
                Y[ay][ax] = v2f{fmaxf(sv.x, kLeaky * sv.x), fmaxf(sv.y, kLeaky * sv.y)};
            }
        }
        if constexpr (FUSE) {
            if (fused) {
                const float wl = a.last_w[cout0];
                v2f P[16];
#pragma unroll
                for (int i = 0; i < 16; ++i) P[i] = Y[i >> 2][i & 3] * wl;
                row_reduce_scatter_step<8, 0x140>(P, (cl & 8) != 0);
                row_reduce_scatter_step<4, 0x141>(P, (cl & 4) != 0);
                row_reduce_scatter_step<2, 0x1B>(P, (cl & 2) != 0);
                row_reduce_scatter_step<1, 0xB1>(P, (cl & 1) != 0);
                part[rp] = P[0];
                continue;
            }
        }
#pragma unroll
        for (int e = 0; e < 2; ++e) {
            const int t = 16 * th + 4 * tg + 2 * rp + e;
            const int tr = t / TC;
            const int py = STK ? 4 * (tr % (TR / 2)) : 4 * tr, px = 4 * (t % TC);
            const int gy = ty0 + py, gx = tx0 + px;
            const unsigned base = (gx < a.W) ? (unsigned)(((gy * a.W + gx) * a.Cout + cout0) * 4) : OOB;
            const unsigned rowb = (unsigned)(a.W * a.Cout * 4);
#pragma unroll
            for (int ay = 0; ay < 4; ++ay)
#pragma unroll
                for (int ax = 0; ax < 4; ++ax) {
                    const float val = e == 0 ? Y[ay][ax].x : Y[ay][ax].y;
                    __builtin_amdgcn_raw_buffer_store_b32(__builtin_bit_cast(unsigned, val), rdst, base + ay * rowb, ax * a.Cout * 4, 0);
                }
            if (a.pooled != nullptr) {
                const int qy = gy >> 1, qx = gx >> 1;
                const unsigned pbase = (qx < Wp) ? (unsigned)(((qy * Wp + qx) * a.Cout + cout0) * 4) : OOB;
                const unsigned prowb = (unsigned)(Wp * a.Cout * 4);
#pragma unroll
                for (int wy = 0; wy < 2; ++wy)
#pragma unroll
                    for (int wx = 0; wx < 2; ++wx) {
                        const v2f mx = __builtin_elementwise_max(__builtin_elementwise_max(Y[2 * wy][2 * wx], Y[2 * wy][2 * wx + 1]),
                                                                 __builtin_elementwise_max(Y[2 * wy + 1][2 * wx], Y[2 * wy + 1][2 * wx + 1]));
                        const float val = e == 0 ? mx.x : mx.y;
                        __builtin_amdgcn_raw_buffer_store_b32(__builtin_bit_cast(unsigned, val), rpool, pbase + wy * prowb, wx * a.Cout * 4, 0);
                    }
            }
        }
    }
    if constexpr (FUSE) {
        if (fused) {
            const int cq = cb & 1, lane = 16 * tg + cl;
            float4* const x4 = reinterpret_cast<float4*>(xch) + th * 64 + lane;
            if (cq == 1) *x4 = make_float4(part[0].x, part[0].y, part[1].x, part[1].y);
            __syncthreads();
            if (cq == 0) {
                const float4 o = *x4;
                const float sum[4] = {part[0].x + o.x, part[0].y + o.y, part[1].x + o.z, part[1].y + o.w};
                const float lb = a.last_b[0];
#pragma unroll
                for (int r = 0; r < 4; ++r) {
                    const int t = 16 * th + 4 * tg + r;
                    const int gy = ty0 + 4 * (t / TC) + (cl >> 2), gx = tx0 + 4 * (t % TC) + (cl & 3);
                    if (gy < a.H && gx < a.W && !nostore) {
                        const size_t qx = ((size_t)n * a.H + gy) * a.W + gx;
                        const float img = a.last_ximg != nullptr ? a.last_ximg[qx] : (a.last_z[qx].x - a.last_u[qx].x);
                        a.last_out[qx] = fminf(fmaxf(img + sum[r] + lb, 0.f), 1.f);
                    }
                }
            }
        }
    }
}

template <int TW, int SRC, bool STK = false, int WN = 2, int MT = 32>
__global__ __launch_bounds__(8 * MT * WN, 2) void conv3x3_wino4_kernel(const ConvArgs a) {
    constexpr int CK = 8 * WN, CKP = CK, LP = CK, PPP = CK / 4, NT_ = 8 * MT * WN;
    constexpr int CKQ = WN == 2 ? CK + 4 : CK + 2;
    constexpr int HCN = CK / 2;
    constexpr int TC = TW / 4, TR = MT / TC;
    constexpr int TH = 4 * TR;
    constexpr int SUBH = STK ? TH / 2 + 2 : 0;
    constexpr int PH = STK ? 2 * SUBH : TH + 2, PW = TW + 2;
    constexpr int ITEMS = PH * PW * PPP;
    static_assert(!STK || (TW == 16 && SRC == SRC_PLAIN && WN == 2 && MT == 32), "stacked slices: 16-wide tiles, plain source");
    static_assert(MT == 32 || (MT == 16 && WN == 2), "16-tile M-blocks: 64-channel workgroups only");
    constexpr int NIT = (ITEMS + NT_ - 1) / NT_;
    constexpr bool UP2 = SRC == SRC_UPCAT;
    constexpr bool FIRST = SRC == SRC_FIRST;
    constexpr int LH = TH / 2 + 3, LW = TW / 2 + 3;
    constexpr int LITEMS = LH * LW * PPP;
    constexpr int NITL = (LITEMS + NT_ - 1) / NT_;
    constexpr bool SPLIT = UP2 && WN == 2;
    constexpr int NH0 = SPLIT ? (NIT + 1) / 2 : NIT;
    constexpr int NRAW = SPLIT ? (NH0 > NITL ? NH0 : NITL) : ((UP2 && NITL > NIT) ? NITL : NIT);
    constexpr int S = CK / 4;
    constexpr int PF = WN == 2 ? 9 : 12;
    constexpr int KEEP = WN == 1 ? 6 : 3;
    constexpr int PLANE = MT * CKP;
    static_assert(SRC == SRC_PLAIN || SRC == SRC_UPCAT || SRC == SRC_FIRST, "pooled sources go through the pooled copy");
    static_assert(!FIRST || (WN == 1 && MT == 32), "fused first layer: the 32-channel variant");
    static_assert(36 % PF == 0 && MT * HCN * 2 == NT_, "one (tile, 2-channel, column group) transform item per thread");

    extern __shared__ __attribute__((aligned(16))) float smem[];
    float* const patch = smem;
    float* const V = smem + ((PH * PW * CKQ + 3) & ~3);
    float* const lowres = V + 36 * PLANE;
    float* const rowT = lowres + LH * LW * LP;
    float* const colT = rowT + 4 * PH;
    constexpr int IW = PW + 3;
    float* const dimg = V + 36 * PLANE;
    float* const mimg = dimg + (PH + 2) * IW;
    float* const wl = mimg + (PH + 2) * IW;
    float* const bl = wl + 18 * 32;
#ifdef PNP_STAMPS
    unsigned long long st_t0 = W4T(), st_setup = 0, st_loop0 = 0, st_commit = 0, st_trans = 0, st_mfma = 0, st_loop1 = 0, st_ew = 0, st_er = 0, st_tmp = 0;
#endif
    const int tid = threadIdx.x, lane = tid & 63;
    const int wid = __builtin_amdgcn_readfirstlane(tid >> 6);
    const int cq = wid / (MT / 16), th = wid % (MT / 16);
    const int tg = lane >> 4, cl = lane & 15;

    const int ny = a.Cout / (32 * WN);
    const int bid = blockIdx.x;
    const int ntl = a.tilesX * a.tilesY * (STK ? (a.N + 1) / 2 : a.N);
    int cby, bt;
    wino4_decode(bid, ny, ntl, a.order, cby, bt);
    if (bt >= ntl) return;
    const int tx0 = (bt % a.tilesX) * TW;
    bt /= a.tilesX;
    const int ty0 = (bt % a.tilesY) * TH;
    const int n = STK ? 2 * (bt / a.tilesY) : bt / a.tilesY;
    const int nsl = STK ? (n + 1 < a.N ? 2 : 1) : 1;
    const bool live0 = !(a.tact != nullptr && a.tact[n] > 0.5f);
    const bool live1 = STK && nsl == 2 && !(a.tact != nullptr && a.tact[n + 1] > 0.5f);
    if (!live0 && !live1) return;
    const int cb = cby * (2 * WN) + cq;
    const int nchunks = a.Cin / CK;

    const int Hs = a.H >> 1, Ws = a.W >> 1;
    const int ylo = UP2 ? ty0 / 2 - 1 : 0;
    const int xlo = UP2 ? (int)(a.rw * (float)(tx0 > 0 ? tx0 - 1 : 0)) : 0;
    const int nskip = UP2 ? a.Cskip / CK : 0;

    constexpr unsigned OOB = 0x80000000u;
    const int cs = UP2 ? a.Cskip : a.Cin;
#ifdef PNP_DIAG
    const bool hot = (a.diag & 2) != 0;
#else
    constexpr bool hot = false;
#endif
    const int ly0 = hot ? 0 : ty0, lx0 = hot ? 0 : tx0, ln = hot ? 0 : n;
    const __amdgpu_buffer_rsrc_t rsrc0 = __builtin_amdgcn_make_buffer_rsrc(
        (void*)(a.src0 + (size_t)ln * a.H * a.W * cs), 0, nsl * a.H * a.W * cs * 4, 0x00020000);
    unsigned voff[NIT];
#pragma unroll
    for (int k = 0; k < NIT; ++k) {
        const int idx = tid + k * NT_;
        const int part = idx % PPP, pp = idx / PPP;
        const int py = pp / PW, px = pp % PW;
        const int sub = STK ? py / SUBH : 0;
        const int gy = STK ? py % SUBH - 1 : ly0 + py - 1, gx = lx0 + px - 1;
        voff[k] = (idx < ITEMS && sub < nsl && gy >= 0 && gy < a.H && gx >= 0 && gx < a.W)
                      ? (unsigned)((((sub * a.H + gy) * a.W + gx) * cs + part * 4) * 4) : OOB;
    }
    const int Cup = a.Cin - a.Cskip;
    const __amdgpu_buffer_rsrc_t rsrc1 = __builtin_amdgcn_make_buffer_rsrc(
        (void*)(UP2 ? a.src1 + (size_t)ln * Hs * Ws * Cup : a.src0), 0, UP2 ? Hs * Ws * Cup * 4 : 0, 0x00020000);
    unsigned voffL[UP2 ? NITL : 1];
    if constexpr (UP2) {
#pragma unroll
        for (int k = 0; k < NITL; ++k) {
            const int idx = tid + k * NT_;
            const int part = idx % PPP, pp = idx / PPP;
            const int sy = (hot ? -1 : ylo) + pp / LW, sx = (hot ? 0 : xlo) + pp % LW;
            voffL[k] = (idx < LITEMS && sy >= 0 && sy < Hs && sx < Ws) ? (unsigned)(((sy * Ws + sx) * Cup + part * 4) * 4) : OOB;
        }
    }
    const int ldst = ((tid / PPP) * CKQ + (tid % PPP) * 4);
    const int ldstL = ((tid / PPP) * LP + (tid % PPP) * 4);
    auto put_patch = [&](int off, float4 v) {
        if constexpr (CKQ % 4 == 0) *reinterpret_cast<float4*>(&patch[off]) = v;
        else { *reinterpret_cast<float2*>(&patch[off]) = make_float2(v.x, v.y); *reinterpret_cast<float2*>(&patch[off + 2]) = make_float2(v.z, v.w); }
    };

    float4 raw[NRAW];
    auto issue = [&](int c, int half = 0) {
        if (UP2 && c >= nskip) {
            if (half != 0) return;
            const int soff = (c * CK - a.Cskip) * 4;
#pragma unroll
            for (int k = 0; k < NITL; ++k)
                raw[k] = __builtin_bit_cast(float4, __builtin_amdgcn_raw_buffer_load_b128(rsrc1, voffL[k], soff, 0));
            return;
        }
        const int soff = c * CK * 4;
        if (half == 0) {
#pragma unroll
            for (int k = 0; k < NH0; ++k)
                raw[k] = __builtin_bit_cast(float4, __builtin_amdgcn_raw_buffer_load_b128(rsrc0, voff[k], soff, 0));
        } else {
#pragma unroll
            for (int k = NH0; k < NIT; ++k)
                raw[k - NH0] = __builtin_bit_cast(float4, __builtin_amdgcn_raw_buffer_load_b128(rsrc0, voff[k], soff, 0));
        }
    };
    auto park = [&](int c, int half = 0) {
        if (UP2 && c >= nskip) {
            if (half != 0) return;
#pragma unroll
            for (int k = 0; k < NITL; ++k) {
                const int idx = tid + k * NT_;
                if (idx < LITEMS) *reinterpret_cast<float4*>(&lowres[ldstL + k * (NT_ / PPP) * LP]) = raw[k];
            }
            return;
        }
        if (half == 0) {
#pragma unroll
            for (int k = 0; k < NH0; ++k) {
                const int idx = tid + k * NT_;
                if (idx < ITEMS) put_patch(ldst + k * (NT_ / PPP) * CKQ, raw[k]);
            }
        } else {
#pragma unroll
            for (int k = NH0; k < NIT; ++k) {
                const int idx = tid + k * NT_;
                if (idx < ITEMS) put_patch(ldst + k * (NT_ / PPP) * CKQ, raw[k - NH0]);
            }
        }
    };
    constexpr int IPAIRS = PW * PPP, IWPG = (IPAIRS + 63) / 64, ING = (NT_ / 64) / IWPG;
    constexpr int IRG = (((PH + ING - 1) / ING) + 1) & ~1;
    constexpr int IK = IRG / 2 + 1;
    static_assert(!UP2 || (ING >= 1 && (PPP & (PPP - 1)) == 0 && TH % 2 == 0), "row groups of whole waves; even tile origin");
    static_assert(!UP2 || ((PH - 1) / 2 + 1 < LH), "the parked region holds every candidate line");
    auto interpolate = [&]() {
        const int ig = wid / IWPG;
        const int it = tid - ig * (IWPG * 64);
        if (ig >= ING || it >= IPAIRS) return;
        const int x = it / PPP, part = it % PPP;
        const int yb = ig * IRG;
        const float4 ct = *reinterpret_cast<const float4*>(&colT[4 * x]);
        const float* const l0 = &lowres[__float_as_int(ct.x) + part * 4 + (yb / 2) * (LW * LP)];
        const float* const l1 = &lowres[__float_as_int(ct.y) + part * 4 + (yb / 2) * (LW * LP)];
        const v2f wx0 = v2f{ct.z, ct.z}, wx1 = v2f{ct.w, ct.w};
        v2f tl[IK], th_[IK];
#pragma unroll
        for (int k = 0; k < IK; ++k) {
            if ((yb / 2 + k) < LH) {
                const float4 pa = *reinterpret_cast<const float4*>(l0 + k * (LW * LP)), pb = *reinterpret_cast<const float4*>(l1 + k * (LW * LP));
                tl[k] = __builtin_elementwise_fma(wx0, v2f{pa.x, pa.y}, wx1 * v2f{pb.x, pb.y});
                th_[k] = __builtin_elementwise_fma(wx0, v2f{pa.z, pa.w}, wx1 * v2f{pb.z, pb.w});
            } else { tl[k] = v2f{0.f, 0.f}; th_[k] = v2f{0.f, 0.f}; }
        }
        const int pdst = ((yb * PW + x) * CKQ) + part * 4;
#pragma unroll
        for (int j = 0; j < IRG; ++j) {
            if (yb + j < PH) {
                const float4 rw = *reinterpret_cast<const float4*>(&rowT[4 * (yb + j)]);
                const v2f wa = v2f{rw.x, rw.x}, wb = v2f{rw.y, rw.y};
                const int k = j >> 1;
                const v2f olo = __builtin_elementwise_fma(wa, tl[k], wb * tl[k + 1]);
                const v2f ohi = __builtin_elementwise_fma(wa, th_[k], wb * th_[k + 1]);
                put_patch(pdst + j * (PW * CKQ), make_float4(olo.x, olo.y, ohi.x, ohi.y));
            }
        }
    };
    bool first_interior = false;
    int fbase[FIRST ? NIT : 1];
    if constexpr (FIRST) {
        first_interior = ty0 >= 2 && ty0 + TH + 2 <= a.H && tx0 >= 2 && tx0 + TW + 2 <= a.W;
        const float sg = a.first_sigma[n];
        for (int i = tid; i < (PH + 2) * (PW + 2); i += NT_) {
            const int r = i / (PW + 2), q = i % (PW + 2);
            const int gy = ty0 - 2 + r, gx = tx0 - 2 + q;
            float d = 0.f, m = 0.f;
            if (gy >= 0 && gy < a.H && gx >= 0 && gx < a.W) {
                const size_t qx = ((size_t)n * a.H + gy) * a.W + gx;
                d = a.last_ximg != nullptr ? a.last_ximg[qx] : (a.last_z[qx].x - a.last_u[qx].x);
                m = 1.f;
            }
            dimg[r * IW + q] = d;
            mimg[r * IW + q] = m;
        }
        for (int i = tid; i < 32 * 18; i += NT_) {
            const int ch = i / 18, t = i % 18;
            wl[t * 32 + ch] = a.first_w[i] * (t >= 9 ? sg : 1.f);
        }
        if (tid < 32) {
            float sc = 0.f;
#pragma unroll
            for (int t = 9; t < 18; ++t) sc += a.first_w[tid * 18 + t] * sg;
            bl[tid] = a.first_b[tid];
            bl[32 + tid] = a.first_b[tid] + sc;
        }
#pragma unroll
        for (int k = 0; k < NIT; ++k) {
            const int pp = (tid + k * NT_) / PPP;
            fbase[k] = (tid + k * NT_ < ITEMS) ? (pp / PW) * IW + pp % PW : 0;
        }
        __syncthreads();
    }
    auto first_patch = [&](int c) {
        if constexpr (FIRST) {
            const int part = tid % PPP;
            const float* const wq = wl + CK * c + 4 * part;
            const f32x4 b4 = *reinterpret_cast<const f32x4*>(bl + (first_interior ? 32 : 0) + CK * c + 4 * part);
            f32x4 acc[NIT];
#pragma unroll
            for (int k = 0; k < NIT; ++k) acc[k] = b4;
#pragma unroll
            for (int t = 0; t < 9; ++t) {
                const f32x4 w4 = *reinterpret_cast<const f32x4*>(wq + t * 32);
#pragma unroll
                for (int k = 0; k < NIT; ++k) acc[k] = __builtin_elementwise_fma(w4, f32x4(dimg[fbase[k] + (t / 3) * IW + t % 3]), acc[k]);
            }
            if (!first_interior) {
#pragma unroll
                for (int t = 0; t < 9; ++t) {
                    const f32x4 w4 = *reinterpret_cast<const f32x4*>(wq + (9 + t) * 32);
#pragma unroll
                    for (int k = 0; k < NIT; ++k) acc[k] = __builtin_elementwise_fma(w4, f32x4(mimg[fbase[k] + (t / 3) * IW + t % 3]), acc[k]);
                }
            }
#pragma unroll
            for (int k = 0; k < NIT; ++k) {
                const int idx = tid + k * NT_;
                if (idx < ITEMS) {
                    const float in = first_interior ? 1.f : mimg[fbase[k] + IW + 1];
                    const f32x4 v = in * __builtin_elementwise_max(acc[k], kLeaky * acc[k]);
                    put_patch((idx / PPP) * CKQ + part * 4, make_float4(v[0], v[1], v[2], v[3]));
                }
            }
        }
    };
    if constexpr (UP2) {
        if (tid < PH + PW) {
            const bool isrow = tid < PH;
            const int pq = isrow ? tid : tid - PH;
            const int g = (isrow ? ty0 : tx0) + pq - 1;
            float4 e = make_float4(0.f, 0.f, 0.f, 0.f);
            if (g >= 0 && g < (isrow ? a.H : a.W)) {
                const float sc = (isrow ? a.rh : a.rw) * (float)g;
                const int i0 = (int)sc;
                const int i1 = i0 + (i0 < (isrow ? Hs : Ws) - 1 ? 1 : 0);
                const float l = fminf(fmaxf(sc - (float)i0, 0.f), 1.f);
                if (isrow) {
                    const int s0 = ylo + (pq >> 1);
                    const float w0 = 1.f - l, w1 = l;
                    e.x = (i0 == s0 ? w0 : 0.f) + (i1 == s0 ? w1 : 0.f);
                    e.y = (i0 == s0 + 1 ? w0 : 0.f) + (i1 == s0 + 1 ? w1 : 0.f);
                } else {
                    e = make_float4(__int_as_float((i0 - xlo) * LP), __int_as_float((i1 - xlo) * LP), 1.f - l, l);
                }
            }
            *reinterpret_cast<float4*>(&(isrow ? rowT : colT)[4 * pq]) = e;
        }
    }
    if constexpr (FIRST) first_patch(0);
    else {
        issue(0); park(0);
        if constexpr (SPLIT) { issue(0, 1); park(0, 1); }
    }

    auto swz = [](int t16, int g) { return WN == 2 ? (g ^ ((4 - (t16 >> 2)) & 3)) : (g ^ ((t16 >> 3) << 1)); };
    const int hc = tid % HCN, tq = (tid / HCN) % MT;
    const int tj = wid / (NT_ / 128);
    const int trow = tq / TC;
    const int wrow = STK ? (trow / (TR / 2)) * SUBH + 4 * (trow % (TR / 2)) : 4 * trow;
    const int win = (wrow * PW + 4 * (tq % TC)) * CKQ + 2 * hc;
    const int vout = WN == 2 ? tq * CKP + 4 * swz(tq & 15, hc >> 1) + 2 * (hc & 1)
                             : tq * CKP + 2 * swz(tq & 15, hc);

    f32x4 acc[36];
#pragma unroll
    for (int k = 0; k < 36; ++k) acc[k] = f32x4{0.f, 0.f, 0.f, 0.f};

    typedef typename std::conditional<WN == 2, float4, float2>::type frag_t;
    const size_t stream = (size_t)nchunks * 36 * 64 + kW4Tail / S;
    const __amdgpu_buffer_rsrc_t rB = __builtin_amdgcn_make_buffer_rsrc(
        (void*)(reinterpret_cast<const frag_t*>(a.wpack) + (size_t)cb * stream), 0, (int)(stream * sizeof(frag_t)), 0x00020000);
    const int boff = lane * (int)sizeof(frag_t);
    const frag_t* const bptr = reinterpret_cast<const frag_t*>(a.wpack) + (size_t)cb * stream + lane;
    auto bfrag = [&](const frag_t* bp, int f0, int i) -> frag_t {
        if constexpr (!UP2) return bp[i * 64];
        else if constexpr (WN == 2) return __builtin_bit_cast(frag_t, __builtin_amdgcn_raw_buffer_load_b128(rB, boff, (f0 + i) * (64 * 16), 0));
        else return __builtin_bit_cast(frag_t, __builtin_amdgcn_raw_buffer_load_b64(rB, boff, (f0 + i) * (64 * 8), 0));
    };
    frag_t bq[PF];
#pragma unroll
    for (int p = 0; p < KEEP; ++p) bq[p] = bfrag(bptr, 0, p);
    const int aoff = (16 * th + cl) * CKP + S * swz(cl, tg);

#ifdef PNP_STAMPS
    st_setup = W4T();
    st_loop0 = st_setup;
#endif
    for (int c = 0; c < nchunks; ++c) {
#ifdef PNP_STAMPS
        st_tmp = W4T();
#endif
        __syncthreads();
        if (UP2 && c >= nskip) {
            if constexpr (NT_ == 256) __builtin_amdgcn_s_setprio(3);
            interpolate();
            if constexpr (NT_ == 256) __builtin_amdgcn_s_setprio(0);
            __syncthreads();
        }
#ifdef PNP_STAMPS
        { const unsigned long long t = W4T(); st_commit += t - st_tmp; st_tmp = t; }
#endif

        if constexpr (WN == 1 && !FIRST) { if (c + 1 < nchunks) issue(c + 1); }
        __builtin_amdgcn_sched_barrier(0);
        if constexpr (NT_ == 256) __builtin_amdgcn_s_setprio(3);
        if (tj == 0) wino4_input_transform<0, PW, CKQ, PLANE>(patch + win, V + vout);
        else wino4_input_transform<1, PW, CKQ, PLANE>(patch + win, V + vout);
        if constexpr (NT_ == 256) __builtin_amdgcn_s_setprio(0);
        __builtin_amdgcn_sched_barrier(0);
        const frag_t* bp = bptr + (size_t)c * 36 * 64;
        const int bf0 = c * 36;
#pragma unroll
        for (int p = KEEP; p < PF; ++p) bq[p] = bfrag(bp, bf0, p);
        if constexpr (WN == 2) { if (c + 1 < nchunks) issue(c + 1); }
        __syncthreads();
#ifdef PNP_STAMPS
        { const unsigned long long t = W4T(); st_trans += t - st_tmp; st_tmp = t; }
#endif

        frag_t ar[3];
        ar[0] = *reinterpret_cast<const frag_t*>(&V[aoff]);
        ar[1] = *reinterpret_cast<const frag_t*>(&V[PLANE + aoff]);
#pragma unroll
        for (int xi = 0; xi < 36; ++xi) {
            if (xi + 2 < 36) ar[(xi + 2) % 3] = *reinterpret_cast<const frag_t*>(&V[(xi + 2) * PLANE + aoff]);
            __builtin_amdgcn_sched_barrier(0);
            const frag_t a0 = ar[xi % 3], b0 = bq[xi % PF];
            acc[xi] = __builtin_amdgcn_mfma_f32_16x16x4f32(a0.x, b0.x, acc[xi], 0, 0, 0);
            acc[xi] = __builtin_amdgcn_mfma_f32_16x16x4f32(a0.y, b0.y, acc[xi], 0, 0, 0);
            if constexpr (WN == 2) {
                acc[xi] = __builtin_amdgcn_mfma_f32_16x16x4f32(a0.z, b0.z, acc[xi], 0, 0, 0);
                acc[xi] = __builtin_amdgcn_mfma_f32_16x16x4f32(a0.w, b0.w, acc[xi], 0, 0, 0);
            }
            __builtin_amdgcn_sched_barrier(0);
            if constexpr (SPLIT) {
                if (xi == 17 && c + 1 < nchunks) { park(c + 1, 0); issue(c + 1, 1); }
            }
#ifdef PNP_DIAG
            if ((a.diag & 4) && (xi & 1)) continue;
#endif
            if (xi + PF < 36 + KEEP) bq[xi % PF] = bfrag(bp, bf0, xi + PF);
        }
#ifdef PNP_STAMPS
        { const unsigned long long t = W4T(); st_mfma += t - st_tmp; }
#endif
        if (c + 1 < nchunks) {
            if constexpr (FIRST) first_patch(c + 1);
            else park(c + 1, SPLIT ? 1 : 0);
        }
    }
#ifdef PNP_STAMPS
    st_loop1 = W4T();
    st_tmp = st_loop1;
#endif

    wino4_epilogue<TW, STK, MT, WN == 1 && MT == 32 && SRC == SRC_PLAIN>(a, acc, n, th, tg, cl, cb, tx0, ty0, STK ? (th == 0 ? live0 : live1) : true, smem);
#ifdef PNP_STAMPS
    {
        const int w = (int)blockIdx.x - (int)(gridDim.x / 2);
        if (tid == 0 && w >= 0 && w < W4_WGS && a.stamp_slot < W4_SLOTS) {
            unsigned long long* o = g_w4_stamps + ((size_t)a.stamp_slot * W4_WGS + w) * W4_N;
            const unsigned long long te = W4T();
            o[0] = 1; o[1] = st_setup - st_t0; o[2] = st_commit; o[3] = st_trans; o[4] = st_mfma; o[5] = st_loop1 - st_loop0;
            o[6] = te - st_tmp; o[7] = 0; o[8] = te - st_loop1; o[9] = te - st_t0; o[10] = (unsigned long long)nchunks;
        }
    }
#endif
}

template <int TW, bool STK>
__global__ __launch_bounds__(512, 2) void conv3x3_wino4p_kernel(const ConvArgs a) {
    constexpr int CK = 16, CKP = 16, PPP = 4, NT_ = 512, S = 4;
    constexpr int TC = TW / 4, TR = 32 / TC;
    constexpr int TH = 4 * TR;
    constexpr int SUBH = STK ? TH / 2 + 2 : 0;
    constexpr int PH = STK ? 2 * SUBH : TH + 2, PW = TW + 2;
    constexpr int NPIX = PH * PW, ITEMS = NPIX * PPP;
    constexpr int NIT = (ITEMS + NT_ - 1) / NT_;
    constexpr int PLSZ = ((NPIX * 4 + 15) / 16) * 16 + 4;
    constexpr int PATCH = 4 * PLSZ;
    constexpr int PF = 12, KEEP = 3;
    constexpr int PLANE = 32 * CKP;
    constexpr unsigned OOB = 0x80000000u;
    static_assert(!STK || TW == 16, "stacked slices: 16-wide tiles");
    static_assert((2 * PATCH + 36 * PLANE) * 4 <= 160 * 1024, "two patch copies + V in one CU's LDS");

    extern __shared__ __attribute__((aligned(16))) float smem[];
    float* const patch = smem;
    float* const V = smem + 2 * PATCH;
#ifdef PNP_STAMPS
    unsigned long long st_t0 = W4T(), st_setup = 0, st_loop0 = 0, st_commit = 0, st_trans = 0, st_mfma = 0, st_loop1 = 0, st_tmp = 0;
#endif
    const int tid = threadIdx.x, lane = tid & 63;
    const int wid = __builtin_amdgcn_readfirstlane(tid >> 6);
    const int grp = wid >> 2, cq = wid & 3;
    const int th = grp;
    const int tg = lane >> 4, cl = lane & 15;

    const int ny = a.Cout / 64;
    const int bid = blockIdx.x;
    const int ntl = a.tilesX * a.tilesY * (STK ? (a.N + 1) / 2 : a.N);
    int cby, bt;
    wino4_decode(bid, ny, ntl, a.order, cby, bt);
    if (bt >= ntl) return;
    const int tx0 = (bt % a.tilesX) * TW;
    bt /= a.tilesX;
    const int ty0 = (bt % a.tilesY) * TH;
    const int n = STK ? 2 * (bt / a.tilesY) : bt / a.tilesY;
    const int nsl = STK ? (n + 1 < a.N ? 2 : 1) : 1;
    const bool live0 = !(a.tact != nullptr && a.tact[n] > 0.5f);
    const bool live1 = STK && nsl == 2 && !(a.tact != nullptr && a.tact[n + 1] > 0.5f);
    if (!live0 && !live1) return;
    const int cb = cby * 4 + cq;
    const int nchunks = a.Cin / CK;

    const __amdgpu_buffer_rsrc_t rsrc0 = __builtin_amdgcn_make_buffer_rsrc(
        (void*)(a.src0 + (size_t)n * a.H * a.W * a.Cin), 0, nsl * a.H * a.W * a.Cin * 4, 0x00020000);
    unsigned voff[NIT];
#pragma unroll
    for (int k = 0; k < NIT; ++k) {
        const int idx = tid + k * NT_;
        const int part = idx % PPP, pp = idx / PPP;
        const int py = pp / PW, px = pp % PW;
        const int sub = STK ? py / SUBH : 0;
        const int gy = STK ? py % SUBH - 1 : ty0 + py - 1, gx = tx0 + px - 1;
        voff[k] = (idx < ITEMS && sub < nsl && gy >= 0 && gy < a.H && gx >= 0 && gx < a.W)
                      ? (unsigned)((((sub * a.H + gy) * a.W + gx) * a.Cin + part * 4) * 4) : OOB;
    }
    const int ldst = (tid & 3) * PLSZ + (tid >> 2) * 4;
    float4 raw[NIT];
    auto issue = [&](int c) {
        const int soff = c * CK * 4;
#pragma unroll
        for (int k = 0; k < NIT; ++k)
            raw[k] = __builtin_bit_cast(float4, __builtin_amdgcn_raw_buffer_load_b128(rsrc0, voff[k], soff, 0));
    };
    auto park = [&](int c) {
        float* const dst = patch + (c & 1) * PATCH + ldst;
#pragma unroll
        for (int k = 0; k < NIT; ++k)
            if (tid + k * NT_ < ITEMS) *reinterpret_cast<float4*>(&dst[k * (NT_ / PPP) * 4]) = raw[k];
    };

    auto swz = [](int t16, int g) { return g ^ ((4 - (t16 >> 2)) & 3); };
    const int tgi = tid & 255;
    const int hc = tgi & 7, t16 = (tgi >> 3) & 15;
    const int tj = (wid >> 1) & 1;
    const int tq = 16 * grp + t16;
    const int trow = tq / TC;
    const int wrow = STK ? (trow / (TR / 2)) * SUBH + 4 * (trow % (TR / 2)) : 4 * trow;
    const int win = (hc >> 1) * PLSZ + (wrow * PW + 4 * (tq % TC)) * 4 + 2 * (hc & 1);
    const int vout = tq * CKP + 4 * swz(t16, hc >> 1) + 2 * (hc & 1);

    f32x4 acc[36];
#pragma unroll
    for (int k = 0; k < 36; ++k) acc[k] = f32x4{0.f, 0.f, 0.f, 0.f};

    const size_t stream = (size_t)nchunks * 36 * 64 + kW4Tail / S;
    const float4* const bptr = reinterpret_cast<const float4*>(a.wpack) + (size_t)cb * stream + lane;
    float4 bq[PF];
#pragma unroll
    for (int p = 0; p < KEEP; ++p) bq[p] = bptr[p * 64];
    const int aoff = (16 * th + cl) * CKP + 4 * swz(cl, tg);

    constexpr bool PARK_T = !STK;
    issue(0);
    park(0);
    if constexpr (!PARK_T) { if (grp == 1 && nchunks > 1) { issue(1); park(1); } }
#ifdef PNP_STAMPS
    st_setup = W4T();
    st_loop0 = st_setup;
#endif
    if (grp == 1) __syncthreads();
    for (int c = 0; c < nchunks; ++c) {
#ifdef PNP_STAMPS
        st_tmp = W4T();
#endif
        __syncthreads();
#ifdef PNP_STAMPS
        { const unsigned long long t = W4T(); st_commit += t - st_tmp; st_tmp = t; }
#endif
        if constexpr (PARK_T) { if (c + 1 < nchunks) issue(c + 1); }
        __builtin_amdgcn_s_setprio(3);
        {
            const float* const w = patch + (c & 1) * PATCH + win;
            if (tj == 0) wino4_input_transform<0, PW, 4, PLANE>(w, V + vout);
            else wino4_input_transform<1, PW, 4, PLANE>(w, V + vout);
        }
        __builtin_amdgcn_s_setprio(0);
        __builtin_amdgcn_sched_barrier(0);
        const float4* bp = bptr + (size_t)c * 36 * 64;
#pragma unroll
        for (int p = KEEP; p < PF; ++p) bq[p] = bp[p * 64];
        const int nx = c + 1 + grp;
        if constexpr (PARK_T) { if (c + 1 < nchunks) park(c + 1); }
        else { if (nx < nchunks) issue(nx); }
        __syncthreads();
#ifdef PNP_STAMPS
        { const unsigned long long t = W4T(); st_trans += t - st_tmp; st_tmp = t; }
#endif

        float4 ar[3];
        ar[0] = *reinterpret_cast<const float4*>(&V[aoff]);
        ar[1] = *reinterpret_cast<const float4*>(&V[PLANE + aoff]);
#pragma unroll
        for (int xi = 0; xi < 36; ++xi) {
            if (xi + 2 < 36) ar[(xi + 2) % 3] = *reinterpret_cast<const float4*>(&V[(xi + 2) * PLANE + aoff]);
            __builtin_amdgcn_sched_barrier(0);
            const float4 a0 = ar[xi % 3], b0 = bq[xi % PF];
            acc[xi] = __builtin_amdgcn_mfma_f32_16x16x4f32(a0.x, b0.x, acc[xi], 0, 0, 0);
            acc[xi] = __builtin_amdgcn_mfma_f32_16x16x4f32(a0.y, b0.y, acc[xi], 0, 0, 0);
            acc[xi] = __builtin_amdgcn_mfma_f32_16x16x4f32(a0.z, b0.z, acc[xi], 0, 0, 0);
            acc[xi] = __builtin_amdgcn_mfma_f32_16x16x4f32(a0.w, b0.w, acc[xi], 0, 0, 0);
            __builtin_amdgcn_sched_barrier(0);
#ifdef PNP_DIAG
            if ((a.diag & 4) && (xi & 1)) continue;
#endif
            if (xi + PF < 36 + KEEP) bq[xi % PF] = bp[(xi + PF) * 64];
        }
#ifdef PNP_STAMPS
        { const unsigned long long t = W4T(); st_mfma += t - st_tmp; }
#endif
        if constexpr (!PARK_T) { if (nx < nchunks) park(nx); }
    }
    if (grp == 0) __syncthreads();
#ifdef PNP_STAMPS
    st_loop1 = W4T();
    st_tmp = st_loop1;
#endif

    wino4_epilogue<TW, STK>(a, acc, n, th, tg, cl, cb, tx0, ty0, STK ? (th == 0 ? live0 : live1) : true);
#ifdef PNP_STAMPS
    {
        const int w = (int)blockIdx.x - (int)(gridDim.x / 2);
        if (tid == 0 && w >= 0 && w < W4_WGS && a.stamp_slot < W4_SLOTS) {
            unsigned long long* o = g_w4_stamps + ((size_t)a.stamp_slot * W4_WGS + w) * W4_N;
            const unsigned long long te = W4T();
            o[0] = 1; o[1] = st_setup - st_t0; o[2] = st_commit; o[3] = st_trans; o[4] = st_mfma; o[5] = st_loop1 - st_loop0;
            o[6] = te - st_tmp; o[7] = 0; o[8] = te - st_loop1; o[9] = te - st_t0; o[10] = (unsigned long long)nchunks;
        }
    }
#endif
}

template <int TW, bool STK>
static hipError_t launch_wino4p_inst(const ConvArgs& a, const WinoPlan& p, hipStream_t s) {
    constexpr int TC = TW / 4, TR = 32 / TC, TH = 4 * TR;
    constexpr int NPIX = (STK ? TH + 4 : TH + 2) * (TW + 2);
    constexpr int PLSZ = ((NPIX * 4 + 15) / 16) * 16 + 4;
    constexpr size_t lds = ((size_t)2 * 4 * PLSZ + (size_t)36 * 32 * 16) * sizeof(float);
    auto kern = conv3x3_wino4p_kernel<TW, STK>;
    static DeviceOnce cap;
    if (hipError_t e = raise_lds_cap((const void*)kern, (int)lds, cap); e != hipSuccess) return e;
    const int ntiles = p.tiles_x * p.tiles_y * (STK ? (a.N + 1) / 2 : a.N), ny = a.Cout / 64;
    dim3 grid((unsigned)(((ntiles + 7) / 8) * 8 * ny));
    hipLaunchKernelGGL(kern, grid, dim3(512), lds, s, a);
    return hipGetLastError();
}

template <int TW, int SRC, bool STK = false, int WN = 2, int MT = 32>
static hipError_t launch_wino4_inst(const ConvArgs& a, const WinoPlan& p, hipStream_t s) {
    constexpr int CK = 8 * WN, CKP = CK, CKQ = WN == 2 ? CK + 4 : CK + 2, TC = TW / 4, TR = MT / TC, TH = 4 * TR;
    constexpr size_t patch_f = (((size_t)(STK ? TH + 4 : TH + 2) * (TW + 2) * CKQ + 3) / 4) * 4;
    constexpr size_t lowres_f = SRC == SRC_UPCAT ? (size_t)(TH / 2 + 3) * (TW / 2 + 3) * CK + 4 * (TH + 2 + TW + 2) : 0;
    constexpr size_t first_f = SRC == SRC_FIRST ? (size_t)2 * (TH + 4) * (TW + 5) + 18 * 32 + 64 : 0;
    constexpr size_t lds = (patch_f + (size_t)36 * MT * CKP + lowres_f + first_f) * sizeof(float);
    static_assert(lds <= (WN == 2 && MT == 32 ? 160 : 80) * 1024, "one (8 waves) / two (4 waves) workgroups per CU");
    if (p.th != TH || p.tw != TW) return hipErrorInvalidValue;
    auto kern = conv3x3_wino4_kernel<TW, SRC, STK, WN, MT>;
    static DeviceOnce cap;
    if (hipError_t e = raise_lds_cap((const void*)kern, (int)lds, cap); e != hipSuccess) return e;
    const int ntiles = p.tiles_x * p.tiles_y * (STK ? (a.N + 1) / 2 : a.N), ny = a.Cout / (32 * WN);
    dim3 grid((unsigned)(((ntiles + 7) / 8) * 8 * ny));
    hipLaunchKernelGGL(kern, grid, dim3(8 * MT * WN), lds, s, a);
    return hipGetLastError();
}

hipError_t launch_conv3x3_winograd4(const ConvArgs& a0, const WinoPlan& p, int src_mode, hipStream_t s) {
    if (!p.use || p.algo != 4 || a0.Cout % p.bn || a0.Cin % p.ck || (src_mode == SRC_UPCAT && a0.Cskip % p.ck) || a0.W % 4) return hipErrorInvalidValue;
    if (a0.last_w != nullptr && !(p.bn == 32 && p.mt == 32 && src_mode == SRC_PLAIN)) return hipErrorInvalidValue;
    ConvArgs a = a0;
    a.tilesX = p.tiles_x;
    a.tilesY = p.tiles_y;
    a.order = p.order;
#ifdef PNP_STAMPS
    a.stamp_slot = g_w4_slot++;
#endif
    if (p.bn == 32) {
        if (p.ck != 8 || p.stack) return hipErrorInvalidValue;
        if (p.tw == 32 && src_mode == SRC_PLAIN) return launch_wino4_inst<32, SRC_PLAIN, false, 1>(a, p, s);
        if (p.tw == 32 && src_mode == SRC_UPCAT) return launch_wino4_inst<32, SRC_UPCAT, false, 1>(a, p, s);
        if (p.tw == 32 && src_mode == SRC_FIRST) return launch_wino4_inst<32, SRC_FIRST, false, 1>(a, p, s);
        if (p.tw == 16 && src_mode == SRC_FIRST) return launch_wino4_inst<16, SRC_FIRST, false, 1>(a, p, s);
        if (p.tw == 16 && src_mode == SRC_PLAIN) return launch_wino4_inst<16, SRC_PLAIN, false, 1>(a, p, s);
        if (p.tw == 16 && src_mode == SRC_UPCAT) return launch_wino4_inst<16, SRC_UPCAT, false, 1>(a, p, s);
        return hipErrorInvalidValue;
    }
    if (p.ck != 16) return hipErrorInvalidValue;
    if (p.mt == 16) {
        if (p.stack) return hipErrorInvalidValue;
        if (p.tw == 32 && src_mode == SRC_PLAIN) return launch_wino4_inst<32, SRC_PLAIN, false, 2, 16>(a, p, s);
        if (p.tw == 32 && src_mode == SRC_UPCAT) return launch_wino4_inst<32, SRC_UPCAT, false, 2, 16>(a, p, s);
        if (p.tw == 16 && src_mode == SRC_PLAIN) return launch_wino4_inst<16, SRC_PLAIN, false, 2, 16>(a, p, s);
        if (p.tw == 16 && src_mode == SRC_UPCAT) return launch_wino4_inst<16, SRC_UPCAT, false, 2, 16>(a, p, s);
        return hipErrorInvalidValue;
    }
    if (p.phased && src_mode == SRC_PLAIN) {
        if (p.tw == 32 && !p.stack) return launch_wino4p_inst<32, false>(a, p, s);
        if (p.tw == 16) {
            if (p.stack) return a.H == 16 && a.W == 16 ? launch_wino4p_inst<16, true>(a, p, s) : hipErrorInvalidValue;
            return launch_wino4p_inst<16, false>(a, p, s);
        }
        return hipErrorInvalidValue;
    }
    if (p.tw == 32) {
        if (src_mode == SRC_PLAIN) return launch_wino4_inst<32, SRC_PLAIN>(a, p, s);
        if (src_mode == SRC_UPCAT) return launch_wino4_inst<32, SRC_UPCAT>(a, p, s);
    } else if (p.tw == 16) {
        if (p.stack) return src_mode == SRC_PLAIN && a.H == 16 && a.W == 16 ? launch_wino4_inst<16, SRC_PLAIN, true>(a, p, s) : hipErrorInvalidValue;
        if (src_mode == SRC_PLAIN) return launch_wino4_inst<16, SRC_PLAIN>(a, p, s);
        if (src_mode == SRC_UPCAT) return launch_wino4_inst<16, SRC_UPCAT>(a, p, s);
    }
    return hipErrorInvalidValue;
}

}

#ifdef PNP_STAMPS
extern "C" int pnp_debug_stamps4_reset(void) { pnp::g_w4_slot = 0; return 0; }
extern "C" int pnp_debug_stamps4_read(unsigned long long* dst, int slots) {
    return (int)hipMemcpyFromSymbol(dst, HIP_SYMBOL(pnp::g_w4_stamps), (size_t)slots * W4_WGS * W4_N * sizeof(unsigned long long));
}
#endif
```

dt4image_restoration_amd/csrc/winograd_kernels.hip:

```cpp
#include "pnp_internal.h"
#include "conv_staging.h"
#include <cstdlib>

namespace pnp {

#ifdef PNP_STAMPS
#define PNP_STAMP_SLOTS 32
#define PNP_STAMP_WGS 1024
#define PNP_STAMP_N 112
__device__ unsigned long long g_wino_stamps[PNP_STAMP_SLOTS * PNP_STAMP_WGS * PNP_STAMP_N];
static int g_stamp_slot = 0;
#define STAMP() do { if (ns < PNP_STAMP_N) st[ns] = __builtin_amdgcn_s_memtime(); ++ns; } while (0)
#else
#define STAMP() do { } while (0)
#endif

size_t winograd_pack_floats(int cin, int cout) { return (size_t)(cout / 32) * ((size_t)(cin / 8) * 16 * 256 + 2 * 4 * 256); }

void pack_winograd_weights(const float* oihw, int cin, int cout, int ck, float* dst) {
    static const double G[4][3] = {{1, 0, 0}, {0.5, 0.5, 0.5}, {0.5, -0.5, 0.5}, {0, 0, 1}};
    std::vector<float> U((size_t)cout * cin * 16);
    for (int co = 0; co < cout; ++co)
        for (int ci = 0; ci < cin; ++ci) {
            const float* g = oihw + ((size_t)co * cin + ci) * 9;
            double t[4][3];
            for (int i = 0; i < 4; ++i)
                for (int kx = 0; kx < 3; ++kx) t[i][kx] = G[i][0] * g[kx] + G[i][1] * g[3 + kx] + G[i][2] * g[6 + kx];
            for (int i = 0; i < 4; ++i)
                for (int j = 0; j < 4; ++j)
                    U[((size_t)co * cin + ci) * 16 + 4 * i + j] = (float)(t[i][0] * G[j][0] + t[i][1] * G[j][1] + t[i][2] * G[j][2]);
        }
    size_t o = 0;
    for (int cb = 0; cb < cout / 32; ++cb)
        for (int half = 0; half < 2; ++half) {
            for (int ch = 0; ch < cin / ck; ++ch)
                for (int ks = 0; ks < ck / 8; ++ks)
                    for (int k = 0; k < 8; ++k)
                        for (int l = 0; l < 64; ++l)
                            for (int j = 0; j < 4; ++j) {
                                const int co = 32 * cb + (l & 31);
                                const int ci = ck * ch + 8 * ks + 4 * (l >> 5) + j;
                                dst[o++] = U[((size_t)co * cin + ci) * 16 + 8 * half + k];
                            }
            for (int i = 0; i < 4 * 256; ++i) dst[o++] = 0.f;
        }
}


WinoPlan winograd_plan(int N, int H, int W, int Cin, int Cout, int src_mode, const Tuning& t) {
    WinoPlan p{};
    p.use = false;
    p.algo = 1;
    if (t.no_wino || Cin < t.wino_min_cin || Cin % 32 || Cout % 32) return p;
    if (!t.no_f4 && Cin >= t.f4_min_cin && (Cout % 64 == 0 || Cout == 32) && Cin % 16 == 0 && (src_mode == SRC_PLAIN || src_mode == SRC_UPCAT) &&
        W >= 16 && H >= 16 && (W >= 32 || H >= 32 || (W == 16 && H == 16 && src_mode == SRC_PLAIN && N >= 2)) &&
        W % 4 == 0 &&
        (src_mode != SRC_UPCAT || upsample_lines_regular(H))) {
        WinoPlan f{};
        f.algo = 4;
        f.order = (t.f4_order && (long)H * W >= 32 * 32) ? 1 : 0;
        f.tw = W >= 32 ? 32 : 16;
        f.th = f.tw == 32 ? 16 : 32;
        f.bn = 64; f.wm = 1; f.wn = 2; f.ck = 16;
        if (Cout == 32) { f.bn = 32; f.wn = 1; f.ck = 8; }
        f.tiles_x = (W + f.tw - 1) / f.tw;
        f.tiles_y = (H + f.th - 1) / f.th;
        f.stack = (W == 16 && H == 16) ? 1 : 0;
        if (!(f.stack && Cout == 32)) {
            f.mt = 32;
            const bool mt16 = t.f4_mt16 == 0 ? (src_mode == SRC_UPCAT || Cin <= 64) : (t.f4_mt16 == 1 ? false : (t.f4_mt16 == 2 ? src_mode == SRC_UPCAT : true));
            if (f.bn == 64 && mt16 && (f.tw == 32 ? H >= 8 : H >= 16)) {
                f.mt = 16;
                f.th = f.tw == 32 ? 8 : 16;
                f.tiles_y = (H + f.th - 1) / f.th;
                f.stack = 0;
            }
            f.phased = (f.mt == 32 && f.bn == 64 && src_mode == SRC_PLAIN && !t.no_f4_phased) ? 1 : 0;
            const long blocks = (long)f.tiles_x * f.tiles_y * (f.stack ? (N + 1) / 2 : N) * (Cout / f.bn);
            f.use = blocks >= t.wino_min_blocks;
            if (f.use) return f;
        }
    }
    p.tw = W >= 32 ? 32 : (W >= 16 ? 16 : 8);
    const bool big = t.wino_big;
    if (Cout % 128 == 0 && !t.wino_small) { p.wm = 1; p.wn = 4; p.ck = 32; }
    else if (Cout % 64 == 0) { if (big) { p.wm = 2; p.wn = 2; } else { p.wm = 1; p.wn = 2; } p.ck = 16; }
    else { if (big) { p.wm = 4; p.wn = 1; } else { p.wm = 2; p.wn = 1; } p.ck = 8; }
    const int tc = p.tw / 2, tr = 32 / tc;
    p.th = p.wm * 2 * tr;
    p.bn = p.wn * 32;
    p.tiles_x = (W + p.tw - 1) / p.tw;
    p.tiles_y = (H + p.th - 1) / p.th;
    const long blocks = (long)p.tiles_x * p.tiles_y * N * (Cout / p.bn);
    p.use = blocks >= t.wino_min_blocks;
    return p;
}

template <int TW, int WM, int WN, int CK, int SRC>
__global__ __launch_bounds__(WM * WN * 128, 2) void conv3x3_winograd_kernel(const ConvArgs a) {
    constexpr int GW = WM * WN;
    constexpr int NT_ = GW * 128;
    constexpr int CKP = CK + 4;
    constexpr int PPP = CK / 4;
    constexpr int TC = TW / 2, TR = 32 / TC;
    constexpr int TH = WM * 2 * TR;
    constexpr int NTILES = WM * 32;
    constexpr int PWL = TW + 2, PH = TH + 2, PW = PWL;
    constexpr int ITEMS = PH * PWL * PPP;
    constexpr int NIT = (ITEMS + NT_ - 1) / NT_;
    constexpr bool UP2 = SRC == SRC_UPCAT;
    constexpr bool PREFETCH = SRC == SRC_PLAIN || UP2;
    constexpr int LH = TH / 2 + 3, LW = TW / 2 + 3;
    constexpr int LITEMS = LH * LW * PPP;
    constexpr int NITL = (LITEMS + NT_ - 1) / NT_;
    constexpr int NRAW = PREFETCH ? (UP2 && NITL > NIT ? NITL : NIT) : (NIT < 3 ? NIT : 3);
    constexpr int LB = PREFETCH ? NIT : (NIT < 3 ? NIT : 3);
    constexpr int KSC = CK / 8;
    constexpr int PAIRS = 8 * KSC;
    constexpr int PF = 4;
    static_assert((GW == 4 || GW == 2) && NTILES * PPP * 2 == NT_, "one (tile, 4-channel, frequency-half) transform item per thread");

#ifdef PNP_STAMPS
    unsigned long long st[PNP_STAMP_N];
    int ns = 0;
    STAMP();
#endif
    extern __shared__ __attribute__((aligned(16))) float smem[];
    float* const patch = smem;
    float* const V = smem + PH * PW * CKP;
    float* const lowres = V + 16 * NTILES * CKP;

    const int tid = threadIdx.x, lane = tid & 63, wid = tid >> 6;
    const int xh = wid / GW;
    const int wm = (wid % GW) / WN, wn = (wid % GW) % WN;
    const int hh = lane >> 5, li = lane & 31;

    int bt = blockIdx.x;
    const int tx0 = (bt % a.tilesX) * TW;
    bt /= a.tilesX;
    const int ty0 = (bt % a.tilesY) * TH;
    const int n = bt / a.tilesY;
    const int cb = blockIdx.y * WN + wn;
    if (a.tact != nullptr && a.tact[n] > 0.5f) return;
    const int nchunks = a.Cin / CK;

    const int Hs = a.H >> 1, Ws = a.W >> 1;
    const int ylo = UP2 ? (int)(a.rh * (float)(ty0 > 0 ? ty0 - 1 : 0)) : 0;
    const int xlo = UP2 ? (int)(a.rw * (float)(tx0 > 0 ? tx0 - 1 : 0)) : 0;
    const int nskip = UP2 ? a.Cskip / CK : 0;

    float4 raw[NRAW][(SRC == SRC_POOL) ? 4 : 1];
    auto issue = [&](int c, int it0, int cnt) {
        if (UP2 && c >= nskip) {
            const int Cup = a.Cin - a.Cskip;
            const float* base = a.src1 + (size_t)n * Hs * Ws * Cup + (c * CK - a.Cskip);
#pragma unroll
            for (int k = 0; k < NITL; ++k) {
                const int idx = tid + k * NT_;
                const int part = idx % PPP, pp = idx / PPP;
                const int sy = ylo + pp / LW, sx = xlo + pp % LW;
                if (idx < LITEMS && sy < Hs && sx < Ws)
                    raw[k][0] = *reinterpret_cast<const float4*>(base + ((size_t)sy * Ws + sx) * Cup + part * 4);
            }
            return;
        }
#pragma unroll
        for (int k = 0; k < cnt; ++k) {
            const int idx = tid + (it0 + k) * NT_;
            const int part = idx % PPP, pp = idx / PPP;
            const int py = pp / PWL, px = pp % PWL;
            const int gy = ty0 + py - 1, gx = tx0 + px - 1;
            if (idx < ITEMS && gy >= 0 && gy < a.H && gx >= 0 && gx < a.W) {
                if constexpr (SRC == SRC_POOL) {
                    RawPiece<SRC_POOL> r;
                    issue_piece<SRC_POOL>(a, n, gy, gx, c * CK + part * 4, r);
                    raw[k][0] = r.v[0]; raw[k][1] = r.v[1]; raw[k][2] = r.v[2]; raw[k][3] = r.v[3];
                } else {
                    const int cs = UP2 ? a.Cskip : a.Cin;
                    raw[k][0] = *reinterpret_cast<const float4*>(a.src0 + (((size_t)n * a.H + gy) * a.W + gx) * cs + c * CK + part * 4);
                }
            }
        }
    };
    auto commit = [&](int c, int it0, int cnt) {
        if (UP2 && c >= nskip) {
#pragma unroll
            for (int k = 0; k < NITL; ++k) {
                const int idx = tid + k * NT_;
                if (idx < LITEMS) *reinterpret_cast<float4*>(&lowres[(idx / PPP) * CKP + (idx % PPP) * 4]) = raw[k][0];
            }
            __syncthreads();
#pragma unroll
            for (int k = 0; k < NIT; ++k) {
                const int idx = tid + k * NT_;
                const int part = idx % PPP, pp = idx / PPP;
                const int py = pp / PWL, px = pp % PWL;
                const int gy = ty0 + py - 1, gx = tx0 + px - 1;
                if (idx < ITEMS) {
                    float4 v = make_float4(0.f, 0.f, 0.f, 0.f);
                    if (gy >= 0 && gy < a.H && gx >= 0 && gx < a.W) {
                        const float sy = a.rh * (float)gy, sx = a.rw * (float)gx;
                        const int y0 = (int)sy, x0 = (int)sx;
                        const int y1 = y0 + (y0 < Hs - 1 ? 1 : 0), x1 = x0 + (x0 < Ws - 1 ? 1 : 0);
                        const float ly = fminf(fmaxf(sy - (float)y0, 0.f), 1.f), lx = fminf(fmaxf(sx - (float)x0, 0.f), 1.f);
                        const float* r0 = &lowres[((y0 - ylo) * LW - xlo) * CKP + part * 4];
                        const float* r1 = &lowres[((y1 - ylo) * LW - xlo) * CKP + part * 4];
                        v = f4lerp2(*reinterpret_cast<const float4*>(r0 + x0 * CKP), *reinterpret_cast<const float4*>(r0 + x1 * CKP),
                                    *reinterpret_cast<const float4*>(r1 + x0 * CKP), *reinterpret_cast<const float4*>(r1 + x1 * CKP),
                                    1.f - lx, lx, 1.f - ly, ly);
                    }
                    *reinterpret_cast<float4*>(&patch[(py * PW + px) * CKP + part * 4]) = v;
                }
            }
            return;
        }
#pragma unroll
        for (int k = 0; k < cnt; ++k) {
            const int idx = tid + (it0 + k) * NT_;
            const int part = idx % PPP, pp = idx / PPP;
            const int py = pp / PWL, px = pp % PWL;
            const int gy = ty0 + py - 1, gx = tx0 + px - 1;
            if (idx < ITEMS) {
                float4 v = make_float4(0.f, 0.f, 0.f, 0.f);
                if (gy >= 0 && gy < a.H && gx >= 0 && gx < a.W) {
                    if constexpr (SRC == SRC_POOL) v = f4max(f4max(raw[k][0], raw[k][1]), f4max(raw[k][2], raw[k][3]));
                    else v = raw[k][0];
                }
                *reinterpret_cast<float4*>(&patch[(py * PW + px) * CKP + part * 4]) = v;
            }
        }
// ... 249 lines not shown
```

dt4image_restoration_amd/engine.py:

```python
from __future__ import annotations

import ctypes as C
from typing import Dict, Mapping, Optional, Tuple

import numpy as np
import torch

from . import _lib
from .weights import flatten_state_dict

RESIDUAL_COLUMNS = _lib.RESIDUAL_COLUMNS


def _ptr(t: Optional[torch.Tensor]) -> Optional[int]:
    return None if t is None else t.data_ptr()


_episode_counter = 0


def _next_episode() -> int:
    global _episode_counter
    _episode_counter += 1
    return _episode_counter
# ... 258 lines not shown
        return y0, aty0, x0

    def estimate_sens(self, y0: torch.Tensor, acs: Tuple[int, int], window: str = "hann", thresh: float = 0.0, return_rss: bool = False):
        if y0.dim() != 4 or y0.shape[0] != self.n or tuple(y0.shape[-2:]) != (self.h, self.w):
            raise ValueError(f"y0: expected [{self.n},C,{self.h},{self.w}], got {tuple(y0.shape)}")
        coils = int(y0.shape[1])
        y0 = self._chk(y0, torch.complex64, self.n * coils * self.h * self.w, "y0")
        if window not in _lib.SENS_WINDOWS:
            raise ValueError(f"window must be one of {tuple(_lib.SENS_WINDOWS)}, got {window!r}")
        acs_h, acs_w = (int(v) for v in acs)
        sens = torch.empty_like(y0)
        rss = torch.empty((self.n, self.h, self.w), dtype=torch.float32, device=self.device) if return_rss else None
        _lib.check(self.lib.pnp_estimate_sens(self._h, y0.data_ptr(), coils, acs_h, acs_w, _lib.SENS_WINDOWS[window], float(thresh), 0,
                                              sens.data_ptr(), _ptr(rss), self._stream()), "pnp_estimate_sens")
        return (sens, rss) if return_rss else sens

    def espirit_sens(self, y0: torch.Tensor, acs: Tuple[int, int], ksize: int = 6, sv_thresh: float = 0.02, crop: float = 0.9, iters: int = 16,
                     window: str = "hann", thresh: float = 0.0, return_eval: bool = False, return_kernels: bool = False):
        if y0.dim() != 4 or y0.shape[0] != self.n or tuple(y0.shape[-2:]) != (self.h, self.w):
            raise ValueError(f"y0: expected [{self.n},C,{self.h},{self.w}], got {tuple(y0.shape)}")
        coils = int(y0.shape[1])
        y0 = self._chk(y0, torch.complex64, self.n * coils * self.h * self.w, "y0")
        if window not in _lib.SENS_WINDOWS:
            raise ValueError(f"window must be one of {tuple(_lib.SENS_WINDOWS)}, got {window!r}")
        if not 1 <= coils <= _lib.PNP_ESPIRIT_MAX_COILS:
            raise ValueError(f"espirit_sens takes 1..{_lib.PNP_ESPIRIT_MAX_COILS} coils, got {coils}: compress the channels first")
        ksize, iters = int(ksize), int(iters)
        if not 2 <= ksize <= _lib.PNP_ESPIRIT_MAX_KSIZE or coils * ksize * ksize > _lib.PNP_ESPIRIT_MAX_N:
            raise ValueError(f"ksize must be 2..{_lib.PNP_ESPIRIT_MAX_KSIZE} with coils * ksize^2 <= {_lib.PNP_ESPIRIT_MAX_N}, got {ksize} at "
                             f"{coils} coils")
        acs_h, acs_w = (int(v) for v in acs)
        sens = torch.empty_like(y0)
        ev = torch.empty((self.n, self.h, self.w), dtype=torch.float32, device=self.device) if return_eval else None
        d = 2 * ksize - 1
        kern = torch.empty((self.n, coils, coils, d, d), dtype=torch.complex64, device=self.device) if return_kernels else None
        nkept = torch.empty((self.n,), dtype=torch.int32, device=self.device) if return_kernels else None
        _lib.check(self.lib.pnp_espirit_sens(self._h, y0.data_ptr(), coils, acs_h, acs_w, ksize, float(sv_thresh), float(crop), iters,
                                             _lib.SENS_WINDOWS[window], float(thresh), 0, sens.data_ptr(), _ptr(ev), _ptr(kern), _ptr(nkept),
                                             self._stream()), "pnp_espirit_sens")
        out = (sens,) + ((ev,) if return_eval else ()) + ((kern, nkept) if return_kernels else ())
        return out if len(out) > 1 else sens

    def coil_compress_matrix(self, y0: torch.Tensor, acs: Tuple[int, int], return_gram: bool = False):
        if y0.dim() != 4 or y0.shape[0] != self.n or tuple(y0.shape[-2:]) != (self.h, self.w):
            raise ValueError(f"y0: expected [{self.n},C,{self.h},{self.w}], got {tuple(y0.shape)}")
        coils = int(y0.shape[1])
        y0 = self._chk(y0, torch.complex64, self.n * coils * self.h * self.w, "y0")
        acs_h, acs_w = (int(v) for v in acs)
        cmat = torch.empty((self.n, coils, coils), dtype=torch.complex64, device=self.device)
        eig = torch.empty((self.n, coils), dtype=torch.float32, device=self.device)
        gram = torch.empty((self.n, coils, coils), dtype=torch.complex128, device=self.device) if return_gram else None
        _lib.check(self.lib.pnp_coil_compress_matrix(self._h, y0.data_ptr(), coils, acs_h, acs_w, 0, cmat.data_ptr(), eig.data_ptr(),
                                                     _ptr(gram), self._stream()), "pnp_coil_compress_matrix")
        return (cmat, eig, gram) if return_gram else (cmat, eig)

    def coil_compress_apply(self, planes: torch.Tensor, cmat: torch.Tensor, out_coils: int) -> torch.Tensor:
        if planes.dim() != 4 or planes.shape[0] != self.n or tuple(planes.shape[-2:]) != (self.h, self.w):
            raise ValueError(f"planes: expected [{self.n},C,{self.h},{self.w}], got {tuple(planes.shape)}")
        coils = int(planes.shape[1])
        planes = self._chk(planes, torch.complex64, self.n * coils * self.h * self.w, "planes")
        if tuple(cmat.shape) not in ((coils, coils), (1, coils, coils), (self.n, coils, coils)):
            raise ValueError(f"cmat: expected [{coils},{coils}] or [{self.n},{coils},{coils}], got {tuple(cmat.shape)}")
        cmat_n = 1 if cmat.numel() == coils * coils else self.n
        cmat = self._chk(cmat, torch.complex64, cmat_n * coils * coils, "cmat")
        out_coils = int(out_coils)
        if not 1 <= out_coils <= min(coils, _lib.PNP_MC_MAX_COILS):
            raise ValueError(f"out_coils must be 1..{min(coils, _lib.PNP_MC_MAX_COILS)}, got {out_coils}")
        out = torch.empty((self.n, out_coils, self.h, self.w), dtype=torch.complex64, device=self.device)
        _lib.check(self.lib.pnp_coil_compress_apply(self._h, planes.data_ptr(), coils, cmat.data_ptr(), cmat_n, out_coils, out.data_ptr(),
                                                    self._stream()), "pnp_coil_compress_apply")
        return out

    def noise_cov(self, noise: torch.Tensor) -> torch.Tensor:
        if noise.dim() not in (2, 3):
            raise ValueError(f"noise: expected [C,S] or [M,C,S], got {tuple(noise.shape)}")
        m = 1 if noise.dim() == 2 else int(noise.shape[0])
        coils, samples = int(noise.shape[-2]), int(noise.shape[-1])
        noise = self._chk(noise, torch.complex64, m * coils * samples, "noise")
        psi = torch.empty((m, coils, coils), dtype=torch.complex128, device=self.device)
        _lib.check(self.lib.pnp_noise_cov(self._h, noise.data_ptr(), m, coils, samples, 0, psi.data_ptr(), self._stream()), "pnp_noise_cov")
        return psi[0] if noise.dim() == 2 else psi

    def whiten_matrix(self, psi: torch.Tensor) -> Tuple[torch.Tensor, torch.Tensor, torch.Tensor]:
        if psi.dim() not in (2, 3) or psi.shape[-1] != psi.shape[-2]:
            raise ValueError(f"psi: expected [C,C] or [M,C,C], got {tuple(psi.shape)}")
        m = 1 if psi.dim() == 2 else int(psi.shape[0])
        coils = int(psi.shape[-1])
        psi = self._chk(psi, torch.complex128, m * coils * coils, "psi")
        wmat = torch.empty(tuple(psi.shape), dtype=torch.complex64, device=self.device)
        lmat = torch.empty_like(wmat)
        info = torch.empty((m,), dtype=torch.int32, device=self.device)
        _lib.check(self.lib.pnp_whiten_matrix(self._h, psi.data_ptr(), m, coils, 0, wmat.data_ptr(), lmat.data_ptr(), info.data_ptr(),
                                              self._stream()), "pnp_whiten_matrix")
        return wmat, lmat, info

    def whiten_apply(self, planes: torch.Tensor, wmat: torch.Tensor, out: Optional[torch.Tensor] = None) -> torch.Tensor:
        if planes.dim() != 4 or planes.shape[0] != self.n or tuple(planes.shape[-2:]) != (self.h, self.w):
            raise ValueError(f"planes: expected [{self.n},C,{self.h},{self.w}], got {tuple(planes.shape)}")
        coils = int(planes.shape[1])
        planes = self._chk(planes, torch.complex64, self.n * coils * self.h * self.w, "planes")
        if tuple(wmat.shape) not in ((coils, coils), (1, coils, coils), (self.n, coils, coils)):
            raise ValueError(f"wmat: expected [{coils},{coils}] or [{self.n},{coils},{coils}], got {tuple(wmat.shape)}")
        wmat_n = 1 if wmat.numel() == coils * coils else self.n
        wmat = self._chk(wmat, torch.complex64, wmat_n * coils * coils, "wmat")
        if out is None:
            out = torch.empty_like(planes)
        elif tuple(out.shape) != tuple(planes.shape):
            raise ValueError(f"out: expected {tuple(planes.shape)}, got {tuple(out.shape)}")
        out = self._chk(out, torch.complex64, planes.numel(), "out")
        _lib.check(self.lib.pnp_whiten_apply(self._h, planes.data_ptr(), coils, wmat.data_ptr(), wmat_n, out.data_ptr(), self._stream()),
                   "pnp_whiten_apply")
        return out

    def snapshot(self, x: torch.Tensor, z: torch.Tensor, u: torch.Tensor, t_state: Optional[torch.Tensor] = None,
                 out: Optional[torch.Tensor] = None) -> torch.Tensor:
        nhw = self.n * self.h * self.w
        self._chk(x, torch.float32, nhw, "x"); self._chk(z, torch.complex64, nhw, "z"); self._chk(u, torch.complex64, nhw, "u")
        if t_state is not None:
            self._chk(t_state, torch.float32, self.n, "t_state")
        nbytes = self.lib.pnp_snapshot_bytes(self._h)
        if out is None:
            out = torch.empty(nbytes, dtype=torch.uint8, device=self.device)
        elif out.numel() * out.element_size() != nbytes or not out.is_contiguous() or out.device != self.device:
            raise ValueError(f"snapshot buffer must be {nbytes} contiguous bytes on {self.device}")
        _lib.check(self.lib.pnp_snapshot(self._h, x.data_ptr(), z.data_ptr(), u.data_ptr(), _ptr(t_state), out.data_ptr(),
                                         self._stream()), "pnp_snapshot")
        return out

    def restore(self, snap: torch.Tensor, x: torch.Tensor, z: torch.Tensor, u: torch.Tensor,
                t_state: Optional[torch.Tensor] = None) -> None:
        nhw = self.n * self.h * self.w
        self._chk(x, torch.float32, nhw, "x"); self._chk(z, torch.complex64, nhw, "z"); self._chk(u, torch.complex64, nhw, "u")
        if t_state is not None:
            self._chk(t_state, torch.float32, self.n, "t_state")
        if snap.numel() * snap.element_size() != self.lib.pnp_snapshot_bytes(self._h) or not snap.is_contiguous():
            raise ValueError("not a snapshot of this engine")
        _lib.check(self.lib.pnp_restore(self._h, snap.data_ptr(), x.data_ptr(), z.data_ptr(), u.data_ptr(), _ptr(t_state),
                                        self._stream()), "pnp_restore")

    def read_stage(self, which: int) -> torch.Tensor:
        c, hh, ww = C.c_int(), C.c_int(), C.c_int()
        _lib.check(self.lib.pnp_unet_read_stage(self._h, which, None, C.byref(c), C.byref(hh), C.byref(ww), self._stream()),
                   "pnp_unet_read_stage")
        out = torch.empty((self.n, c.value, hh.value, ww.value), dtype=torch.float32, device=self.device)
        _lib.check(self.lib.pnp_unet_read_stage(self._h, which, out.data_ptr(), None, None, None, self._stream()),
                   "pnp_unet_read_stage")
        return out

    def conv_algorithms(self):
        out = (C.c_int32 * _lib.N_LAYERS)()
        _lib.check(self.lib.pnp_conv_algorithms(self._h, out), "pnp_conv_algorithms")
        return list(out)

    def bf16_weight_terms(self) -> int:
        return int(self.lib.pnp_bf16_weight_terms(self._h))

    def profile_reset(self) -> None:
        _lib.check(self.lib.pnp_profile_reset(self._h), "pnp_profile_reset")

    def profile_collect(self) -> Dict[str, Dict[str, float]]:
        ms = (C.c_double * _lib.PROFILE_CLASSES)()
        cnt = (C.c_int64 * _lib.PROFILE_CLASSES)()
        _lib.check(self.lib.pnp_profile_collect(self._h, ms, cnt), "pnp_profile_collect")
        lms = (C.c_double * _lib.N_LAYERS)()
        lcnt = (C.c_int64 * _lib.N_LAYERS)()
        _lib.check(self.lib.pnp_profile_layers(self._h, lms, lcnt), "pnp_profile_layers")
        out = {name: {"ms": ms[i], "launches": int(cnt[i])} for i, name in enumerate(_lib.PROFILE_CLASS_NAMES)}
        out["layers"] = {"ms": list(lms), "launches": [int(v) for v in lcnt]}
        return out
```

include/pnpadmm.h:

```cpp
#ifndef PNPADMM_H
#define PNPADMM_H

#include <stddef.h>
#include <stdint.h>

#ifdef __cplusplus
extern "C" {
#endif

typedef struct pnp_engine* pnp_handle;

typedef enum {
    PNP_OK = 0,
    PNP_ERR_INVALID = -1,
    PNP_ERR_HIP = -2,
    PNP_ERR_STATE = -3,
    PNP_ERR_NOMEM = -4,
    PNP_ERR_INTERNAL = -5
} pnp_status;

typedef struct {
    int32_t n;
    int32_t h, w;
    int32_t device;
    int32_t flags;
} pnp_config;

#define PNP_FLAG_PROFILE 1
#define PNP_FLAG_PROFILE_LAYERS 16
#define PNP_FLAG_NO_DENOISER 2
#define PNP_FLAG_KEEP_STAGES 4
#define PNP_FLAG_BF16_CONVS 8


int pnp_create(const pnp_config* cfg, pnp_handle* out);
int pnp_destroy(pnp_handle h);
const char* pnp_last_error(void);
const char* pnp_version(void);

int pnp_load_unet_weights(pnp_handle h, const float* blob, size_t n_floats);


int pnp_reset(pnp_handle h, const float* x0, const float* y0, const uint8_t* mask, int mask_n,
              float* x, float* z, float* u, void* stream);

int pnp_set_kspace(pnp_handle h, const float* y0, const uint8_t* mask, int mask_n, void* stream);

int pnp_step(pnp_handle h, const float* mu, const float* sigma_d, const float* t_action,
             float* x, float* z, float* u, float* t_state, uint8_t* done, void* stream);


int pnp_denoise(pnp_handle h, const float* x_in, const float* sigma, float* out, void* stream);

#define PNP_TV_MAX_ITERS 64
int pnp_tv_denoise(pnp_handle h, const float* x_in, const float* lam, int iters, float* out, void* stream);

#define PNP_PRIOR_UNET 0
#define PNP_PRIOR_TV   1
int pnp_set_prior(pnp_handle h, int prior, double tv_scale, int tv_iters);
int pnp_get_prior(pnp_handle h, int* prior, double* tv_scale, int* tv_iters);

int pnp_fft2c(pnp_handle h, const float* in, float* out, int batch, int hh, int ww, int inverse, void* stream);

int pnp_prox_dual(pnp_handle h, const float* mu, const float* t_action, const float* x, float* z, float* u,
                  void* stream);

int pnp_psnr(pnp_handle h, const float* x, const float* gt, float* out, void* stream);

#define PNP_SSIM_CLAMP_X 1
int pnp_ssim(pnp_handle h, const float* x, const float* gt, float data_range, float k1, float k2, int radius, int flags,
             float* out, float* map, void* stream);

#define PNP_RES_COLS   6
#define PNP_RES_DELTA  1
#define PNP_RES_DC     2
int pnp_residuals(pnp_handle h, const float* x, const float* z, const float* u, const void* prev, int flags, float* out,
                  void* stream);

int pnp_acquire(pnp_handle h, const float* gt, const uint8_t* mask, int mask_n, double sigma_n, uint64_t seed, int flags,
                float* y0, float* aty0, float* x0, void* stream);

#define PNP_MC_MAX_COILS 32
#define PNP_MC_MAX_CG 64
int pnp_set_kspace_mc(pnp_handle h, const float* y0, const float* sens, int coils, int sens_n, const uint8_t* mask, int mask_n, int cg_iters,
                      void* stream);
int pnp_reset_mc(pnp_handle h, const float* x0, const float* y0, const float* sens, int coils, int sens_n, const uint8_t* mask, int mask_n,
                 int cg_iters, float* x, float* z, float* u, void* stream);
int pnp_mc_coils(pnp_handle h);
int pnp_mc_cg_residual(pnp_handle h, float* out, void* stream);
int pnp_mc_normal(pnp_handle h, const float* p, const float* mu, float* q, void* stream);
int pnp_acquire_mc(pnp_handle h, const float* gt, const float* sens, int coils, int sens_n, const uint8_t* mask, int mask_n, double sigma_n,
                   uint64_t seed, int flags, float* y0, float* aty0, float* x0, void* stream);

#define PNP_SENS_BOX  0
#define PNP_SENS_HANN 1
int pnp_estimate_sens(pnp_handle h, const float* y0, int coils, int acs_h, int acs_w, int window, double thresh, int flags,
                      float* sens, float* rss , void* stream);

#define PNP_CC_MAX_COILS 64
int pnp_coil_compress_matrix(pnp_handle h, const float* y0, int coils, int acs_h, int acs_w, int flags, float* cmat, float* eig,
                             double* gram , void* stream);
int pnp_coil_compress_apply(pnp_handle h, const float* in, int coils, const float* cmat, int cmat_n, int out_coils, float* out, void* stream);

#define PNP_PW_MAX_COILS 64
int pnp_noise_cov(pnp_handle h, const float* noise, int noise_n, int coils, int samples, int flags, double* psi, void* stream);
int pnp_whiten_matrix(pnp_handle h, const double* psi, int psi_n, int coils, int flags, float* wmat, float* lmat ,
                      int32_t* info, void* stream);
int pnp_whiten_apply(pnp_handle h, const float* in, int coils, const float* wmat, int wmat_n, float* out, void* stream);

#define PNP_ESPIRIT_MAX_COILS 16
#define PNP_ESPIRIT_MAX_KSIZE 8
#define PNP_ESPIRIT_MAX_N     512
int pnp_espirit_sens(pnp_handle h, const float* y0, int coils, int acs_h, int acs_w, int ksize, double sv_thresh, double crop, int iters,
                     int window, double thresh, int flags, float* sens, float* eval ,
                     float* kern , int32_t* nkept , void* stream);


size_t pnp_snapshot_bytes(pnp_handle h);
int pnp_snapshot(pnp_handle h, const float* x, const float* z, const float* u, const float* t_state, void* dst,
                 void* stream);
int pnp_restore(pnp_handle h, const void* src, float* x, float* z, float* u, float* t_state, void* stream);


int pnp_unet_read_stage(pnp_handle h, int which, float* dst, int* c, int* hh, int* ww, void* stream);

#define PNP_PROFILE_CLASSES 6
int pnp_profile_reset(pnp_handle h);
int pnp_profile_collect(pnp_handle h, double* total_ms, int64_t* launches);
int pnp_profile_layers(pnp_handle h, double* layer_ms, int64_t* layer_launches);

int pnp_conv_algorithms(pnp_handle h, int32_t* algo28);

int pnp_bf16_weight_terms(pnp_handle h);

size_t pnp_workspace_bytes(pnp_handle h);

#ifdef __cplusplus
}
#endif
#endif
```

Measured before the change: 129.1.

## Add channel-split Winograd F4 kernel for upsample-concat decoder convolutions

```diff
diff --git a/dt4image_restoration_amd/_lib.py b/dt4image_restoration_amd/_lib.py
--- a/dt4image_restoration_amd/_lib.py
+++ b/dt4image_restoration_amd/_lib.py
@@ -83,6 +83,7 @@
     "pnp_profile_collect": (C.c_int, [C.c_void_p, C.POINTER(C.c_double), C.POINTER(C.c_int64)]),
     "pnp_profile_layers": (C.c_int, [C.c_void_p, C.POINTER(C.c_double), C.POINTER(C.c_int64)]),
     "pnp_conv_algorithms": (C.c_int, [C.c_void_p, C.POINTER(C.c_int32)]),
+    "pnp_conv_schedules": (C.c_int, [C.c_void_p, C.POINTER(C.c_int32)]),
     "pnp_bf16_weight_terms": (C.c_int, [C.c_void_p]),
     "pnp_workspace_bytes": (C.c_size_t, [C.c_void_p]),
 }
diff --git a/dt4image_restoration_amd/csrc/conv_kernels.hip b/dt4image_restoration_amd/csrc/conv_kernels.hip
--- a/dt4image_restoration_amd/csrc/conv_kernels.hip
+++ b/dt4image_restoration_amd/csrc/conv_kernels.hip
@@ -729,6 +729,7 @@
     t.no_f4_fused_last = getenv("PNP_NO_F4_FUSED_LAST") != nullptr;
     t.no_f4_fused_first = getenv("PNP_NO_F4_FUSED_FIRST") != nullptr;
     if (const char* v = getenv("PNP_WINO_F4_MT16")) t.f4_mt16 = atoi(v);
+    if (const char* v = getenv("PNP_WINO_F4_CS")) t.f4_cs = atoi(v);
     if (const char* v = getenv("PNP_WINO_F4_ORDER")) t.f4_order = atoi(v) != 0;
     t.bf16_f32_acts = getenv("PNP_BF16_F32_ACTS") != nullptr;
     t.bf16_no_ws = getenv("PNP_BF16_NO_WS") != nullptr;
diff --git a/dt4image_restoration_amd/csrc/denoiser_plan.hip b/dt4image_restoration_amd/csrc/denoiser_plan.hip
--- a/dt4image_restoration_amd/csrc/denoiser_plan.hip
+++ b/dt4image_restoration_amd/csrc/denoiser_plan.hip
@@ -54,11 +54,11 @@
             rec[li - 1].pooled = r.src0 = {kLayers[li - 1].level, SLOT_POOL};
             P.pool_ok[kLayers[li - 1].level] = true;
         }
-        r.wino = winograd_plan(cfg.n, lh, lw, L.cin, L.cout, r.src_mode, tune);
+        r.wino = winograd_plan(cfg.n, lh, lw, L.cin, L.cout, r.src_mode, tune, L.cskip);
         if (li == kTail && r.wino.algo == 4 && !keep_stages && (tune.no_f4_fused_last || r.wino.bn != 32 || r.wino.mt != 32)) {
             Tuning t2 = tune;
             t2.no_f4 = true;
-            r.wino = winograd_plan(cfg.n, lh, lw, L.cin, L.cout, r.src_mode, t2);
+            r.wino = winograd_plan(cfg.n, lh, lw, L.cin, L.cout, r.src_mode, t2, L.cskip);
         }
         const bool ws_ok = !tune.bf16_no_ws && (r.src_mode != SRC_UPCAT || upsample_lines_regular(lh));
         r.conv = conv3x3_plan(cfg.n, lh, lw, L.cin, L.cout, bf16, r.src_mode, ws_ok);
diff --git a/dt4image_restoration_amd/csrc/pnp_capi.hip b/dt4image_restoration_amd/csrc/pnp_capi.hip
--- a/dt4image_restoration_amd/csrc/pnp_capi.hip
+++ b/dt4image_restoration_amd/csrc/pnp_capi.hip
@@ -1347,6 +1347,21 @@
     PNP_API_END("pnp_conv_algorithms")
 }
 
+int pnp_conv_schedules(pnp_handle e, int32_t* sched28) {
+    PNP_API_BEGIN
+    if (!e || !sched28) return fail(PNP_ERR_INVALID, "pnp_conv_schedules: null argument");
+    if (e->cfg.flags & PNP_FLAG_NO_DENOISER) return fail(PNP_ERR_STATE, "pnp_conv_schedules: handle has no denoiser");
+    for (int i = 0; i < N_LAYERS; ++i) {
+        const int at = e->dplan.launch_of[i];
+        sched28[i] = 0;
+        if (at < 0 || e->dplan.family[i] != FAM_WINO4) continue;
+        const WinoPlan& w = e->dplan.launch[at].wino;
+        sched28[i] = w.cs ? 4 : (w.mt == 16 ? 3 : (w.phased ? 2 : 1));
+    }
+    return PNP_OK;
+    PNP_API_END("pnp_conv_schedules")
+}
+
 int pnp_profile_reset(pnp_handle e) {
     PNP_API_BEGIN
     if (!e) return fail(PNP_ERR_INVALID, "null handle");
diff --git a/dt4image_restoration_amd/csrc/pnp_internal.h b/dt4image_restoration_amd/csrc/pnp_internal.h
--- a/dt4image_restoration_amd/csrc/pnp_internal.h
+++ b/dt4image_restoration_amd/csrc/pnp_internal.h
@@ -23,6 +23,7 @@
     bool bf16_f32_acts = false;
     bool bf16_no_holdhi = false;
     bool bf16_w1 = false;
+    int f4_cs = 1;
     int f4_order = 1;
     int splitk_inlaunch = 0;
     bool fft_xcd = false;
@@ -97,9 +98,10 @@
     int stack;
     int mt;
     int phased;
+    int cs;
     int order;
 };
-WinoPlan winograd_plan(int N, int H, int W, int Cin, int Cout, int src_mode, const Tuning& t);
+WinoPlan winograd_plan(int N, int H, int W, int Cin, int Cout, int src_mode, const Tuning& t, int Cskip = 0);
 bool upsample_lines_regular(int H);
 size_t winograd4_pack_floats(int cin, int cout);
 void pack_winograd4_weights(const float* oihw, int cin, int cout, int ck, float* dst);
diff --git a/dt4image_restoration_amd/csrc/winograd4_kernels.hip b/dt4image_restoration_amd/csrc/winograd4_kernels.hip
--- a/dt4image_restoration_amd/csrc/winograd4_kernels.hip
+++ b/dt4image_restoration_amd/csrc/winograd4_kernels.hip
@@ -134,6 +134,72 @@
         cby = slot - lt * ny;
         bt = lt < tpx ? xcd * tpx + lt : ntiles;
     }
+}
+
+template <int PH, int PW, int PPP, int NW>
+struct Wino4Interp {
+    static constexpr int IPAIRS = PW * PPP, IWPG = (IPAIRS + 63) / 64, ING = NW / IWPG;
+    static constexpr int IRG = (((PH + (ING > 0 ? ING : 1) - 1) / (ING > 0 ? ING : 1)) + 1) & ~1;
+    static constexpr int IK = IRG / 2 + 1;
+};
+template <int PH, int PW, int PPP, int LH, int LW, int LP, int NW, int ROWSTEP, class Slot, class Put>
+__device__ __forceinline__ void wino4_interpolate(const float* lowres, const float* rowT, const float* colT, int w, int t, Slot slot, Put put) {
+    typedef Wino4Interp<PH, PW, PPP, NW> G;
+    constexpr int IPAIRS = G::IPAIRS, IWPG = G::IWPG, ING = G::ING, IRG = G::IRG, IK = G::IK;
+    const int ig = w / IWPG;
+    const int it = t - ig * (IWPG * 64);
+    if (ig >= ING || it >= IPAIRS) return;
+    const int x = it / PPP, part = it % PPP;
+    const int yb = ig * IRG;
+    const float4 ct = *reinterpret_cast<const float4*>(&colT[4 * x]);
+    const float* const l0 = &lowres[__float_as_int(ct.x) + part * 4 + (yb / 2) * (LW * LP)];
+    const float* const l1 = &lowres[__float_as_int(ct.y) + part * 4 + (yb / 2) * (LW * LP)];
+    const v2f wx0 = v2f{ct.z, ct.z}, wx1 = v2f{ct.w, ct.w};
+    v2f tl[IK], th_[IK];
+#pragma unroll
+    for (int k = 0; k < IK; ++k) {
+        if ((yb / 2 + k) < LH) {
+            const float4 pa = *reinterpret_cast<const float4*>(l0 + k * (LW * LP)), pb = *reinterpret_cast<const float4*>(l1 + k * (LW * LP));
+            tl[k] = __builtin_elementwise_fma(wx0, v2f{pa.x, pa.y}, wx1 * v2f{pb.x, pb.y});
+            th_[k] = __builtin_elementwise_fma(wx0, v2f{pa.z, pa.w}, wx1 * v2f{pb.z, pb.w});
+        } else { tl[k] = v2f{0.f, 0.f}; th_[k] = v2f{0.f, 0.f}; }
+    }
+    const int pdst = slot(yb, x, part);
+#pragma unroll
+    for (int j = 0; j < IRG; ++j) {
+        if (yb + j < PH) {
+            const float4 rw = *reinterpret_cast<const float4*>(&rowT[4 * (yb + j)]);
+            const v2f wa = v2f{rw.x, rw.x}, wb = v2f{rw.y, rw.y};
+            const int k = j >> 1;
+            const v2f olo = __builtin_elementwise_fma(wa, tl[k], wb * tl[k + 1]);
+            const v2f ohi = __builtin_elementwise_fma(wa, th_[k], wb * th_[k + 1]);
+            put(pdst + j * ROWSTEP, make_float4(olo.x, olo.y, ohi.x, ohi.y));
+        }
+    }
+}
+template <int PH, int PW, int LP>
+__device__ __forceinline__ void wino4_upsample_tables(const ConvArgs& a, int tid, int ty0, int tx0, int ylo, int xlo, float* rowT, float* colT) {
+    if (tid >= PH + PW) return;
+    const int Hs = a.H >> 1, Ws = a.W >> 1;
+    const bool isrow = tid < PH;
+    const int pq = isrow ? tid : tid - PH;
+    const int g = (isrow ? ty0 : tx0) + pq - 1;
+    float4 e = make_float4(0.f, 0.f, 0.f, 0.f);
+    if (g >= 0 && g < (isrow ? a.H : a.W)) {
+        const float sc = (isrow ? a.rh : a.rw) * (float)g;
+        const int i0 = (int)sc;
+        const int i1 = i0 + (i0 < (isrow ? Hs : Ws) - 1 ? 1 : 0);
+        const float l = fminf(fmaxf(sc - (float)i0, 0.f), 1.f);
+        if (isrow) {
+            const int s0 = ylo + (pq >> 1);
+            const float w0 = 1.f - l, w1 = l;
+            e.x = (i0 == s0 ? w0 : 0.f) + (i1 == s0 ? w1 : 0.f);
+            e.y = (i0 == s0 + 1 ? w0 : 0.f) + (i1 == s0 + 1 ? w1 : 0.f);
+        } else {
+            e = make_float4(__int_as_float((i0 - xlo) * LP), __int_as_float((i1 - xlo) * LP), 1.f - l, l);
+        }
+    }
+    *reinterpret_cast<float4*>(&(isrow ? rowT : colT)[4 * pq]) = e;
 }
 
 template <int CTRL>
@@ -427,42 +493,12 @@
             }
         }
     };
-    constexpr int IPAIRS = PW * PPP, IWPG = (IPAIRS + 63) / 64, ING = (NT_ / 64) / IWPG;
-    constexpr int IRG = (((PH + ING - 1) / ING) + 1) & ~1;
-    constexpr int IK = IRG / 2 + 1;
-    static_assert(!UP2 || (ING >= 1 && (PPP & (PPP - 1)) == 0 && TH % 2 == 0), "row groups of whole waves; even tile origin");
+    typedef Wino4Interp<PH, PW, PPP, NT_ / 64> IG;
+    static_assert(!UP2 || (IG::ING >= 1 && (PPP & (PPP - 1)) == 0 && TH % 2 == 0), "row groups of whole waves; even tile origin");
     static_assert(!UP2 || ((PH - 1) / 2 + 1 < LH), "the parked region holds every candidate line");
     auto interpolate = [&]() {
-        const int ig = wid / IWPG;
-        const int it = tid - ig * (IWPG * 64);
-        if (ig >= ING || it >= IPAIRS) return;
-        const int x = it / PPP, part = it % PPP;
-        const int yb = ig * IRG;
-        const float4 ct = *reinterpret_cast<const float4*>(&colT[4 * x]);
-        const float* const l0 = &lowres[__float_as_int(ct.x) + part * 4 + (yb / 2) * (LW * LP)];
-        const float* const l1 = &lowres[__float_as_int(ct.y) + part * 4 + (yb / 2) * (LW * LP)];
-        const v2f wx0 = v2f{ct.z, ct.z}, wx1 = v2f{ct.w, ct.w};
-        v2f tl[IK], th_[IK];
-#pragma unroll
-        for (int k = 0; k < IK; ++k) {
-            if ((yb / 2 + k) < LH) {
-                const float4 pa = *reinterpret_cast<const float4*>(l0 + k * (LW * LP)), pb = *reinterpret_cast<const float4*>(l1 + k * (LW * LP));
-                tl[k] = __builtin_elementwise_fma(wx0, v2f{pa.x, pa.y}, wx1 * v2f{pb.x, pb.y});
-                th_[k] = __builtin_elementwise_fma(wx0, v2f{pa.z, pa.w}, wx1 * v2f{pb.z, pb.w});
-            } else { tl[k] = v2f{0.f, 0.f}; th_[k] = v2f{0.f, 0.f}; }
-        }
-        const int pdst = ((yb * PW + x) * CKQ) + part * 4;
-#pragma unroll
-        for (int j = 0; j < IRG; ++j) {
-            if (yb + j < PH) {
-                const float4 rw = *reinterpret_cast<const float4*>(&rowT[4 * (yb + j)]);
-                const v2f wa = v2f{rw.x, rw.x}, wb = v2f{rw.y, rw.y};
-                const int k = j >> 1;
-                const v2f olo = __builtin_elementwise_fma(wa, tl[k], wb * tl[k + 1]);
-                const v2f ohi = __builtin_elementwise_fma(wa, th_[k], wb * th_[k + 1]);
-                put_patch(pdst + j * (PW * CKQ), make_float4(olo.x, olo.y, ohi.x, ohi.y));
-            }
-        }
+        wino4_interpolate<PH, PW, PPP, LH, LW, LP, NT_ / 64, PW * CKQ>(lowres, rowT, colT, wid, tid,
+            [](int y, int x, int part) { return ((y * PW + x) * CKQ) + part * 4; }, [&](int off, float4 v) { put_patch(off, v); });
     };
     bool first_interior = false;
     int fbase[FIRST ? NIT : 1];
@@ -533,27 +569,7 @@
         }
     };
     if constexpr (UP2) {
-        if (tid < PH + PW) {
-            const bool isrow = tid < PH;
-            const int pq = isrow ? tid : tid - PH;
-            const int g = (isrow ? ty0 : tx0) + pq - 1;
-            float4 e = make_float4(0.f, 0.f, 0.f, 0.f);
-            if (g >= 0 && g < (isrow ? a.H : a.W)) {
-                const float sc = (isrow ? a.rh : a.rw) * (float)g;
-                const int i0 = (int)sc;
-                const int i1 = i0 + (i0 < (isrow ? Hs : Ws) - 1 ? 1 : 0);
-                const float l = fminf(fmaxf(sc - (float)i0, 0.f), 1.f);
-                if (isrow) {
-                    const int s0 = ylo + (pq >> 1);
-                    const float w0 = 1.f - l, w1 = l;
-                    e.x = (i0 == s0 ? w0 : 0.f) + (i1 == s0 ? w1 : 0.f);
-                    e.y = (i0 == s0 + 1 ? w0 : 0.f) + (i1 == s0 + 1 ? w1 : 0.f);
-                } else {
-                    e = make_float4(__int_as_float((i0 - xlo) * LP), __int_as_float((i1 - xlo) * LP), 1.f - l, l);
-                }
-            }
-            *reinterpret_cast<float4*>(&(isrow ? rowT : colT)[4 * pq]) = e;
-        }
+        wino4_upsample_tables<PH, PW, LP>(a, tid, ty0, tx0, ylo, xlo, rowT, colT);
     }
     if constexpr (FIRST) first_patch(0);
     else {
@@ -851,6 +867,259 @@
 #endif
 }
 
+template <int TW, int SRC>
+__global__ __launch_bounds__(512, 2) void conv3x3_wino4c_kernel(const ConvArgs a) {
+    constexpr int CK = 16, CKP = 16, PPP = 4, NT_ = 512, S = 4, MT = 16;
+    constexpr bool UP2 = SRC == SRC_UPCAT;
+    static_assert(SRC == SRC_PLAIN || SRC == SRC_UPCAT, "plain or upsample + concat source");
+    constexpr int TC = TW / 4, TR = MT / TC;
+    constexpr int TH = 4 * TR;
+    constexpr int PH = TH + 2, PW = TW + 2;
+    constexpr int NPIX = PH * PW, ITEMS = NPIX * PPP;
+    constexpr int NIT = (ITEMS + NT_ - 1) / NT_;
+    constexpr int PLSZ = ((NPIX * 4 + 15) / 16) * 16 + 4;
+    constexpr int PATCH = 4 * PLSZ;
+    constexpr int PF = 12, KEEP = 3;
+    constexpr int PLANE = MT * CKP;
+    constexpr int VSZ = 36 * PLANE;
+    constexpr unsigned OOB = 0x80000000u;
+    static_assert(NIT == 3 && ITEMS <= NIT * NT_, "three staging items per thread");
+    constexpr int LP = CK;
+    constexpr int LH = TH / 2 + 3, LW = TW / 2 + 3;
+    constexpr int LITEMS = LH * LW * PPP, NITL = (LITEMS + NT_ - 1) / NT_;
+    constexpr int LOWRES = LH * LW * LP;
+    static_assert((2 * PATCH + 2 * VSZ + (UP2 ? 2 * LOWRES + 4 * (PH + PW) : 0)) * 4 <= 160 * 1024, "everything in one CU's LDS");
+
+    extern __shared__ __attribute__((aligned(16))) float smem[];
+    float* const patch = smem;
+    float* const V = smem + 2 * PATCH;
+    float* const lowres = V + 2 * VSZ;
+    float* const rowT = lowres + 2 * LOWRES;
+    float* const colT = rowT + 4 * PH;
+#ifdef PNP_STAMPS
+    unsigned long long st_t0 = W4T(), st_setup = 0, st_loop0 = 0, st_commit = 0, st_trans = 0, st_mfma = 0, st_loop1 = 0, st_tmp = 0;
+#endif
+    const int tid = threadIdx.x, lane = tid & 63;
+    const int wid = __builtin_amdgcn_readfirstlane(tid >> 6);
+    const int half = wid >> 2;
+    const int tg = lane >> 4, cl = lane & 15;
+
+    const int ny = a.Cout / 128;
+    const int bid = blockIdx.x;
+    const int ntl = a.tilesX * a.tilesY * a.N;
+    int cby, bt;
+    wino4_decode(bid, ny, ntl, a.order, cby, bt);
+    if (bt >= ntl) return;
+    const int tx0 = (bt % a.tilesX) * TW;
+    bt /= a.tilesX;
+    const int ty0 = (bt % a.tilesY) * TH;
+    const int n = bt / a.tilesY;
+    if (a.tact != nullptr && a.tact[n] > 0.5f) return;
+    const int cb = cby * 8 + wid;
+    const int nchunks = a.Cin / CK;
+    const int cs = UP2 ? a.Cskip : a.Cin;
+    const int nskip = UP2 ? a.Cskip / CK : nchunks;
+    const int Hs = a.H >> 1, Ws = a.W >> 1;
+    const int ylo = UP2 ? ty0 / 2 - 1 : 0;
+    const int xlo = UP2 ? (int)(a.rw * (float)(tx0 > 0 ? tx0 - 1 : 0)) : 0;
+
+    const __amdgpu_buffer_rsrc_t rsrc0 = __builtin_amdgcn_make_buffer_rsrc(
+        (void*)(a.src0 + (size_t)n * a.H * a.W * cs), 0, a.H * a.W * cs * 4, 0x00020000);
+    unsigned voff[NIT];
+#pragma unroll
+    for (int k = 0; k < NIT; ++k) {
+        const int idx = tid + k * NT_;
+        const int part = idx % PPP, pp = idx / PPP;
+        const int gy = ty0 + pp / PW - 1, gx = tx0 + pp % PW - 1;
+        voff[k] = (idx < ITEMS && gy >= 0 && gy < a.H && gx >= 0 && gx < a.W) ? (unsigned)(((gy * a.W + gx) * cs + part * 4) * 4) : OOB;
+    }
+    const int ldst = (tid & 3) * PLSZ + (tid >> 2) * 4;
+    float4 raw[NIT];
+    const int Cup = a.Cin - a.Cskip;
+    const __amdgpu_buffer_rsrc_t rsrc1 = __builtin_amdgcn_make_buffer_rsrc(
+        (void*)(UP2 ? a.src1 + (size_t)n * Hs * Ws * Cup : a.src0), 0, UP2 ? Hs * Ws * Cup * 4 : 0, 0x00020000);
+    unsigned voffL[UP2 ? NITL : 1];
+    float4 rawL[UP2 ? NITL : 1];
+    if constexpr (UP2) {
+#pragma unroll
+        for (int k = 0; k < NITL; ++k) {
+            const int idx = tid + k * NT_;
+            const int part = idx % PPP, pp = idx / PPP;
+            const int sy = ylo + pp / LW, sx = xlo + pp % LW;
+            voffL[k] = (idx < LITEMS && sy >= 0 && sy < Hs && sx < Ws) ? (unsigned)(((sy * Ws + sx) * Cup + part * 4) * 4) : OOB;
+        }
+    }
+    const int ldstL = (tid >> 2) * LP + (tid & 3) * 4;
+    auto issueL = [&](int c) {
+        if constexpr (UP2) {
+            const int soff = (c * CK - a.Cskip) * 4;
+#pragma unroll
+            for (int k = 0; k < NITL; ++k)
+                rawL[k] = __builtin_bit_cast(float4, __builtin_amdgcn_raw_buffer_load_b128(rsrc1, voffL[k], soff, 0));
+        }
+    };
+    auto parkL = [&](int c) {
+        if constexpr (UP2) {
+            float* const dst = lowres + (c & 1) * LOWRES + ldstL;
+#pragma unroll
+            for (int k = 0; k < NITL; ++k)
+                if (tid + k * NT_ < LITEMS) *reinterpret_cast<float4*>(&dst[k * (NT_ / PPP) * LP]) = rawL[k];
+        }
+    };
+    static_assert(Wino4Interp<PH, PW, PPP, 4>::ING >= 1 && TH % 2 == 0 && (PH - 1) / 2 + 1 < LH, "row groups of whole waves; even tile origin; every candidate line parked");
+    auto interpolate = [&](int c) {
+        if constexpr (UP2) {
+            float* const pdst = patch + (c & 1) * PATCH;
+            wino4_interpolate<PH, PW, PPP, LH, LW, LP, 4, PW * 4>(lowres + (c & 1) * LOWRES, rowT, colT, wid & 3, tid & 255,
+                [](int y, int x, int part) { return part * PLSZ + (y * PW + x) * 4; }, [&](int off, float4 v) { *reinterpret_cast<float4*>(&pdst[off]) = v; });
+        }
+    };
+    if constexpr (UP2) {
+        wino4_upsample_tables<PH, PW, LP>(a, tid, ty0, tx0, ylo, xlo, rowT, colT);
+    }
+    auto issue = [&](int c) {
+        const int soff = c * CK * 4;
+#pragma unroll
+        for (int k = 0; k < NIT; ++k)
+            raw[k] = __builtin_bit_cast(float4, __builtin_amdgcn_raw_buffer_load_b128(rsrc0, voff[k], soff, 0));
+    };
+    auto park = [&](int c) {
+        float* const dst = patch + (c & 1) * PATCH + ldst;
+#pragma unroll
+        for (int k = 0; k < NIT; ++k)
+            if (tid + k * NT_ < ITEMS) *reinterpret_cast<float4*>(&dst[k * (NT_ / PPP) * 4]) = raw[k];
+    };
+
+    auto swz = [](int t16, int g) { return g ^ ((4 - (t16 >> 2)) & 3); };
+    const int tgi = tid & 255;
+    const int hc = tgi & 7, t16 = (tgi >> 3) & 15;
+    const int tj = (wid >> 1) & 1;
+    const int win = (hc >> 1) * PLSZ + (4 * (t16 / TC) * PW + 4 * (t16 % TC)) * 4 + 2 * (hc & 1);
+    const int vout = t16 * CKP + 4 * swz(t16, hc >> 1) + 2 * (hc & 1);
+    auto transform = [&](int c) {
+        const float* const w = patch + (c & 1) * PATCH + win;
+        float* const v = V + (c & 1) * VSZ + vout;
+        if (tj == 0) wino4_input_transform<0, PW, 4, PLANE>(w, v);
+        else wino4_input_transform<1, PW, 4, PLANE>(w, v);
+    };
+
+    f32x4 acc[36];
+#pragma unroll
+    for (int k = 0; k < 36; ++k) acc[k] = f32x4{0.f, 0.f, 0.f, 0.f};
+
+    const size_t stream = (size_t)nchunks * 36 * 64 + kW4Tail / S;
+    const __amdgpu_buffer_rsrc_t rB = __builtin_amdgcn_make_buffer_rsrc(
+        (void*)(reinterpret_cast<const float4*>(a.wpack) + (size_t)cb * stream), 0, (int)(stream * sizeof(float4)), 0x00020000);
+    const int boff = lane * (int)sizeof(float4);
+    const float4* const bptr = reinterpret_cast<const float4*>(a.wpack) + (size_t)cb * stream + lane;
+    auto bfrag = [&](const float4* bp, int f0, int i) -> float4 {
+        if constexpr (!UP2) return bp[i * 64];
+        else return __builtin_bit_cast(float4, __builtin_amdgcn_raw_buffer_load_b128(rB, boff, (f0 + i) * (64 * 16), 0));
+    };
+    float4 bq[PF];
+#pragma unroll
+    for (int p = 0; p < KEEP; ++p) bq[p] = bfrag(bptr, 0, p);
+    const int aoff = cl * CKP + 4 * swz(cl, tg);
+
+    issue(0);
+    park(0);
+    if (nchunks > 1) issue(1);
+    __syncthreads();
+    if (half == 1) transform(0);
+    if (nchunks > 1) park(1);
+#ifdef PNP_STAMPS
+    st_setup = W4T();
+    st_loop0 = st_setup;
+#endif
+    for (int c = 0; c < nchunks; ++c) {
+#ifdef PNP_STAMPS
+        st_tmp = W4T();
+#endif
+        __syncthreads();
+#ifdef PNP_STAMPS
+        { const unsigned long long t = W4T(); st_commit += t - st_tmp; st_tmp = t; }
+#endif
+        if (half == (c & 1)) {
+            if (c + 1 < nchunks) {
+                __builtin_amdgcn_s_setprio(3);
+                transform(c + 1);
+                __builtin_amdgcn_s_setprio(0);
+            }
+        } else if (UP2 && c + 2 >= nskip && c + 2 < nchunks) {
+            __builtin_amdgcn_s_setprio(3);
+            interpolate(c + 2);
+            __builtin_amdgcn_s_setprio(0);
+        }
+        __builtin_amdgcn_sched_barrier(0);
+        const float4* bp = bptr + (size_t)c * 36 * 64;
+        const int bf0 = c * 36;
+#pragma unroll
+        for (int p = KEEP; p < PF; ++p) bq[p] = bfrag(bp, bf0, p);
+        if (c + 2 < nskip) issue(c + 2);
+        if (UP2 && c + 3 >= nskip && c + 3 < nchunks) issueL(c + 3);
+#ifdef PNP_STAMPS
+        { const unsigned long long t = W4T(); st_trans += t - st_tmp; st_tmp = t; }
+#endif
+
+        const float* const Vc = V + (c & 1) * VSZ + aoff;
+        float4 ar[3];
+        ar[0] = *reinterpret_cast<const float4*>(&Vc[0]);
+        ar[1] = *reinterpret_cast<const float4*>(&Vc[PLANE]);
+#pragma unroll
+        for (int xi = 0; xi < 36; ++xi) {
+            if (xi + 2 < 36) ar[(xi + 2) % 3] = *reinterpret_cast<const float4*>(&Vc[(xi + 2) * PLANE]);
+            __builtin_amdgcn_sched_barrier(0);
+            const float4 a0 = ar[xi % 3], b0 = bq[xi % PF];
+            acc[xi] = __builtin_amdgcn_mfma_f32_16x16x4f32(a0.x, b0.x, acc[xi], 0, 0, 0);
+            acc[xi] = __builtin_amdgcn_mfma_f32_16x16x4f32(a0.y, b0.y, acc[xi], 0, 0, 0);
+            acc[xi] = __builtin_amdgcn_mfma_f32_16x16x4f32(a0.z, b0.z, acc[xi], 0, 0, 0);
+            acc[xi] = __builtin_amdgcn_mfma_f32_16x16x4f32(a0.w, b0.w, acc[xi], 0, 0, 0);
+            __builtin_amdgcn_sched_barrier(0);
+            if (xi + PF < 36 + KEEP) bq[xi % PF] = bfrag(bp, bf0, xi + PF);
+        }
+#ifdef PNP_STAMPS
+        { const unsigned long long t = W4T(); st_mfma += t - st_tmp; }
+#endif
+        if (c + 2 < nskip) park(c + 2);
+        if (UP2 && c + 3 >= nskip && c + 3 < nchunks) parkL(c + 3);
+    }
+#ifdef PNP_STAMPS
+    st_loop1 = W4T();
+    st_tmp = st_loop1;
+#endif
+
+    wino4_epilogue<TW, false, 16>(a, acc, n, 0, tg, cl, cb, tx0, ty0, true);
+#ifdef PNP_STAMPS
+    {
+        const int w = (int)blockIdx.x - (int)(gridDim.x / 2);
+        if (tid == 0 && w >= 0 && w < W4_WGS && a.stamp_slot < W4_SLOTS) {
+            unsigned long long* o = g_w4_stamps + ((size_t)a.stamp_slot * W4_WGS + w) * W4_N;
+            const unsigned long long te = W4T();
+            o[0] = 1; o[1] = st_setup - st_t0; o[2] = st_commit; o[3] = st_trans; o[4] = st_mfma; o[5] = st_loop1 - st_loop0;
+            o[6] = te - st_tmp; o[7] = 0; o[8] = te - st_loop1; o[9] = te - st_t0; o[10] = (unsigned long long)nchunks;
+        }
+    }
+#endif
+}
+
+template <int TW, int SRC>
+static hipError_t launch_wino4c_inst(const ConvArgs& a, const WinoPlan& p, hipStream_t s) {
+    constexpr int TC = TW / 4, TR = 16 / TC, TH = 4 * TR;
+    constexpr int NPIX = (TH + 2) * (TW + 2);
+    constexpr int PLSZ = ((NPIX * 4 + 15) / 16) * 16 + 4;
+    constexpr size_t lowres_f = SRC == SRC_UPCAT ? (size_t)2 * (TH / 2 + 3) * (TW / 2 + 3) * 16 + 4 * (TH + 2 + TW + 2) : 0;
+    constexpr size_t lds = ((size_t)2 * 4 * PLSZ + (size_t)2 * 36 * 16 * 16 + lowres_f) * sizeof(float);
+    if (p.th != TH || p.tw != TW) return hipErrorInvalidValue;
+    if (SRC == SRC_UPCAT && a.Cskip < 3 * 16) return hipErrorInvalidValue;
+    auto kern = conv3x3_wino4c_kernel<TW, SRC>;
+    static DeviceOnce cap;
+    if (hipError_t e = raise_lds_cap((const void*)kern, (int)lds, cap); e != hipSuccess) return e;
+    const int ntiles = p.tiles_x * p.tiles_y * a.N, ny = a.Cout / 128;
+    dim3 grid((unsigned)(((ntiles + 7) / 8) * 8 * ny));
+    hipLaunchKernelGGL(kern, grid, dim3(512), lds, s, a);
+    return hipGetLastError();
+}
+
 template <int TW, bool STK>
 static hipError_t launch_wino4p_inst(const ConvArgs& a, const WinoPlan& p, hipStream_t s) {
     constexpr int TC = TW / 4, TR = 32 / TC, TH = 4 * TR;
@@ -905,6 +1174,14 @@
         return hipErrorInvalidValue;
     }
     if (p.ck != 16) return hipErrorInvalidValue;
+    if (p.cs) {
+        if (p.bn != 128 || p.mt != 16 || p.stack) return hipErrorInvalidValue;
+        if (p.tw == 32 && src_mode == SRC_PLAIN) return launch_wino4c_inst<32, SRC_PLAIN>(a, p, s);
+        if (p.tw == 32 && src_mode == SRC_UPCAT) return launch_wino4c_inst<32, SRC_UPCAT>(a, p, s);
+        if (p.tw == 16 && src_mode == SRC_PLAIN) return launch_wino4c_inst<16, SRC_PLAIN>(a, p, s);
+        if (p.tw == 16 && src_mode == SRC_UPCAT) return launch_wino4c_inst<16, SRC_UPCAT>(a, p, s);
+        return hipErrorInvalidValue;
+    }
     if (p.mt == 16) {
         if (p.stack) return hipErrorInvalidValue;
         if (p.tw == 32 && src_mode == SRC_PLAIN) return launch_wino4_inst<32, SRC_PLAIN, false, 2, 16>(a, p, s);
diff --git a/dt4image_restoration_amd/csrc/winograd_kernels.hip b/dt4image_restoration_amd/csrc/winograd_kernels.hip
--- a/dt4image_restoration_amd/csrc/winograd_kernels.hip
+++ b/dt4image_restoration_amd/csrc/winograd_kernels.hip
@@ -47,7 +47,8 @@
 }
 
 
-WinoPlan winograd_plan(int N, int H, int W, int Cin, int Cout, int src_mode, const Tuning& t) {
+WinoPlan winograd_plan(int N, int H, int W, int Cin, int Cout, int src_mode, const Tuning& t, int Cskip) {
+    constexpr long kCsMinBlocks = 256;
     WinoPlan p{};
     p.use = false;
     p.algo = 1;
@@ -76,6 +77,19 @@
                 f.stack = 0;
             }
             f.phased = (f.mt == 32 && f.bn == 64 && src_mode == SRC_PLAIN && !t.no_f4_phased) ? 1 : 0;
+            const bool cs_can = f.bn == 64 && Cout % 128 == 0 && (src_mode == SRC_PLAIN || (Cskip % 16 == 0 && Cskip >= 48));
+            const int cs_th = f.tw == 32 ? 8 : 16;
+            const long cs_blocks = (long)f.tiles_x * ((H + cs_th - 1) / cs_th) * N * (Cout / 128);
+            const bool cs_rule = src_mode == SRC_UPCAT && cs_blocks >= kCsMinBlocks;
+            if (cs_can && cs_blocks >= t.wino_min_blocks && (t.f4_cs == 2 || (t.f4_cs == 1 && t.f4_mt16 == 0 && !t.no_f4_phased && cs_rule))) {
+                f.cs = 1;
+                f.bn = 128;
+                f.mt = 16;
+                f.th = cs_th;
+                f.tiles_y = (H + f.th - 1) / f.th;
+                f.stack = 0;
+                f.phased = 0;
+            }
             const long blocks = (long)f.tiles_x * f.tiles_y * (f.stack ? (N + 1) / 2 : N) * (Cout / f.bn);
             f.use = blocks >= t.wino_min_blocks;
             if (f.use) return f;
diff --git a/dt4image_restoration_amd/engine.py b/dt4image_restoration_amd/engine.py
--- a/dt4image_restoration_amd/engine.py
+++ b/dt4image_restoration_amd/engine.py
@@ -434,6 +434,11 @@
         _lib.check(self.lib.pnp_conv_algorithms(self._h, out), "pnp_conv_algorithms")
         return list(out)
 
+    def conv_schedules(self):
+        out = (C.c_int32 * _lib.N_LAYERS)()
+        _lib.check(self.lib.pnp_conv_schedules(self._h, out), "pnp_conv_schedules")
+        return list(out)
+
     def bf16_weight_terms(self) -> int:
         return int(self.lib.pnp_bf16_weight_terms(self._h))
 
diff --git a/include/pnpadmm.h b/include/pnpadmm.h
--- a/include/pnpadmm.h
+++ b/include/pnpadmm.h
@@ -131,6 +131,8 @@
 
 int pnp_conv_algorithms(pnp_handle h, int32_t* algo28);
 
+int pnp_conv_schedules(pnp_handle h, int32_t* sched28);
+
 int pnp_bf16_weight_terms(pnp_handle h);
 
 size_t pnp_workspace_bytes(pnp_handle h);
```

Measured after the change: 130.6, median of 6. 1.2% higher.
